# kylemcdonald/distributed-video-filter

Measured on AMD Instinct MI355X. Metric: frames/sec (1080p RGB invert) at 1/2/4/8 GPUs; kernel HBM GB/s vs peak, higher is better.
Workload: dtype u8; 1 GPU; configs[1]: 1080p RGB invert, batch=32, kernel-only, HBM-resident; global_batch=32, frames_per_rank_step=32, ring_bytes_in_plus_out=2388787200, kernel=invert_stream_kernel<4,nt,nt>, grid 32 WG/CU (vf_kernels.hip)

## Files before the change

### distributed-video-filter_amd/csrc/vf_jpeg.h

```cpp
#pragma once
#include <hip/hip_runtime.h>
#include <stddef.h>
#include <stdint.h>

#include "vf_jpeg_types.h"

namespace vf {
namespace jpeg {


hipError_t scan_u32(const ScanSeg *segs, int nseg, uint32_t max_tiles, const uint32_t *in, uint32_t *out,
                    uint32_t *tsum, uint32_t *totals, bool inclusive, hipStream_t s);
hipError_t scan_i32(const ScanSeg *segs, int nseg, uint32_t max_tiles, const int32_t *in, int32_t *out,
                    int32_t *tsum, int32_t *totals, bool inclusive, hipStream_t s);

hipError_t dec_unstuff_count(const DecSeg *sg, int nseg, uint32_t max_tiles, const uint8_t *in,
                             uint32_t *tile_cnt, hipStream_t s);
hipError_t dec_unstuff_write(const DecSeg *sg, int nseg, uint32_t max_tiles, const uint8_t *in,
                             const uint32_t *tile_off, const uint32_t *us_len, uint8_t *us, hipStream_t s);
hipError_t dec_syncg(int G, const DecSeg *sg, const DecFrame *fr, int nseg, uint32_t max_sub, const uint8_t *us,
                     const uint32_t *us_len, uint64_t *exits, uint32_t *cnts, uint64_t *used, uint64_t *ck,
                     uint32_t *ckrem, uint32_t *changed, int pass, uint32_t warm, int tabs4, hipStream_t s);
hipError_t dec_sync(const DecSeg *sg, const DecFrame *fr, int nseg, uint32_t max_sub, const uint8_t *us, const uint32_t *us_len,
                    const uint64_t *exit_in, uint64_t *exit_out, const uint32_t *cnt_in, uint32_t *cnt_out,
                    uint64_t *used, uint64_t *ck, uint32_t *ckrem, uint32_t *changed, int pass, hipStream_t s);
struct SpecBufs {
  uint64_t *tE;
  uint64_t *tX;
  uint32_t *tXc;
  uint64_t *pX;
  uint32_t *pC;
  uint8_t *wF;
  uint8_t *rE;
  uint32_t *rK;
  uint64_t *qX;
  uint32_t *qC;
  uint8_t *rL;
  uint32_t *stats;
};
constexpr int kSpecLanesMax = 16;
inline uint32_t spec_lanes_host(int bpm) { return bpm <= 1 ? 1u : bpm <= 2 ? 2u : bpm <= 4 ? 4u : bpm <= 8 ? 8u : 16u; }
hipError_t dec_sync_spec(const DecSeg *sg, const DecFrame *fr, int nseg, uint32_t max_wg, const uint8_t *us, const uint32_t *us_len,
                         const SpecBufs &b, uint64_t *exit_out, uint32_t *cnt_out, uint32_t *unresolved,
                         int lsb, hipStream_t s);
hipError_t dec_write(const DecSeg *sg, const DecFrame *fr, int nseg, uint32_t max_sub, const uint8_t *us, const uint32_t *us_len,
                     const uint64_t *exits, const uint32_t *bstart, int16_t *coef, int32_t *dcseq,
                     uint8_t *nmask, hipStream_t s);
hipError_t dec_write4(const DecSeg *sg, const DecFrame *fr, int nseg, uint32_t max_sub, const uint8_t *us,
                      const uint32_t *us_len, const uint64_t *exits, const uint32_t *cnt, const uint64_t *ck,
                      const uint32_t *ckrem, const uint32_t *bstart, int16_t *coef, int32_t *dcseq, uint8_t *nmask,
                      hipStream_t s);
hipError_t dec_idct(const DecFrame *fr, int n, uint32_t max_blocks, const int16_t *coef, const int32_t *dcseq,
                    const uint8_t *nmask, uint8_t *planes, hipStream_t s);
struct LutTable {
  uint32_t w[192];
};
hipError_t dec_color(const DecFrame *fr, int n, int max_w, int max_h, const uint8_t *planes, uint8_t *pix,
                     int bgr, int invert, const EncFrame *efr, int cm, hipStream_t s, const LutTable *lut = nullptr);
hipError_t dec_idct_color422(const DecFrame *fr, int n, int max_w, int max_h, const int16_t *coef,
                             const int32_t *dcseq, const uint8_t *nmask, uint8_t *eplanes, const EncFrame *efr,
                             int invert, int one_row,
                             hipStream_t s,
                             const LutTable *lut = nullptr);

hipError_t enc_fdct(const EncFrame *fr, int n, uint32_t max_blocks, const EncTables *tab, const uint8_t *pix,
                    int16_t *dcq, uint32_t *acbits, uint32_t *acscr, int bgr, int fastdct, int ch, int cv, int planes,
                    hipStream_t s);
hipError_t enc_len(const EncFrame *fr, int n, uint32_t max_blocks, const EncTables *tab, const int16_t *dcq,
                   uint32_t *acbits, uint32_t *bits, uint32_t *pre, hipStream_t s);
hipError_t enc_pack(const EncFrame *fr, int n, uint32_t max_blocks, const uint32_t *pre, const uint32_t *acbits,
                    const uint32_t *acscr, const uint32_t *bitoff, const uint32_t *total_bits, uint8_t *stream,
                    hipStream_t s);
hipError_t enc_ff_count(const EncFrame *fr, int n, uint32_t max_tiles, const uint32_t *total_bits,
                        const uint8_t *stream, uint32_t *tile_cnt, hipStream_t s);
hipError_t enc_ff_write(const EncFrame *fr, int n, uint32_t max_tiles, const uint32_t *total_bits,
                        const uint8_t *stream, const uint32_t *tile_off, const uint32_t *nff,
                        const uint8_t *hdr, uint8_t *pack, uint64_t *out_size, hipStream_t s);

}
}
```

### distributed-video-filter_amd/csrc/vf_jpeg_codec.h

```cpp
#pragma once
#include <hip/hip_runtime.h>

#include <atomic>
#include <condition_variable>
#include <functional>
#include <memory>
#include <mutex>
#include <string>
#include <thread>
#include <vector>

#include "vf_chain_plan.h"
#include "vf_jpeg.h"
#include "vf_jpeg_plan.h"

namespace vf {
namespace jpeg {

constexpr int kOk = 0;
constexpr int kInvalid = -1;
constexpr int kHip = -2;
constexpr int kNoMem = -3;
constexpr int kJpeg = -5;
constexpr int kResync = -100;

constexpr int kFlagFastUpsample = 256;
constexpr int kFlagFastDct = 2048;

struct DevBuf {
  void *p = nullptr;
  size_t cap = 0;
  hipError_t ensure(size_t n);
  template <typename T>
  T *as() const {
    return static_cast<T *>(p);
  }
  ~DevBuf();
};

struct HostBuf {
  void *p = nullptr;
  size_t cap = 0;
  hipError_t ensure(size_t n);
  template <typename T>
  T *as() const {
    return static_cast<T *>(p);
  }
  ~HostBuf();
};

class TaskPool {
 public:
  explicit TaskPool(int nthreads);
  ~TaskPool();
  TaskPool(const TaskPool &) = delete;
  TaskPool &operator=(const TaskPool &) = delete;
  void run(int n, const std::function<void(int)> &fn);

 private:
  void loop();
  void drain();
  std::vector<std::thread> threads_;
  std::mutex mu_;
  std::condition_variable cv_, done_cv_;
  uint64_t gen_ = 0;
  bool stop_ = false;
  int active_ = 0;
  int n_ = 0;
  std::atomic<int> next_{0};
  const std::function<void(int)> *fn_ = nullptr;
};

struct ComputeGate {
  std::mutex mu;
  hipEvent_t last = nullptr;
};

struct ChainSpec {
  chain::Program prog;
  std::vector<uint64_t> masks;
  chain::Buffers bufs;
};

struct Filter {
  enum Kind { kNone, kInvert, kTable, kChain } kind = kInvert;
  LutTable lut = {};
  std::shared_ptr<const ChainSpec> chain;
  bool in_colour() const { return kind == kInvert || kind == kTable; }
  bool between() const { return kind == kChain; }
};

int header_info(const uint8_t *jpeg, size_t size, int *w, int *h, int *subsamp, int *colorspace, std::string *err);
size_t buffer_size(int w, int h, int subsamp);

class Codec {
 public:
  explicit Codec(int device, ComputeGate *gate = nullptr);
  ~Codec();
  Codec(const Codec &) = delete;
  Codec &operator=(const Codec &) = delete;

  int encode(const uint8_t *const *imgs, const int *ws, const int *hs, int n, int pixel_format, int quality,
             int subsamp, int flags, uint8_t *const *outs, const size_t *caps, size_t *sizes, std::string *err);
  int decode(const uint8_t *const *jpegs, const size_t *sizes, int n, int pixel_format, int flags,
             uint8_t *const *outs, const size_t *caps, std::string *err);
  int invert(const uint8_t *const *jpegs, const size_t *sizes, int n, int quality, int subsamp, int flags,
             uint8_t *const *outs, const size_t *caps, size_t *out_sizes, const Filter &filter, std::string *err);
  int submit_invert(const uint8_t *const *jpegs, const size_t *sizes, int n, int quality, int subsamp, int flags,
                    const Filter &filter, std::string *err);
  bool done_invert();
  int wait_invert(size_t *total, std::string *err);
  int fetch_invert(uint8_t *out, size_t cap, size_t *sizes, size_t *offs, std::string *err);
  int scatter_invert(uint8_t *const *outs, const size_t *caps, size_t *sizes, int *placed);
  uint64_t fetch_refills() const { return fetch_refills_; }
  void set_max_pixels(uint64_t v) { max_pixels_ = v ? v : kDefaultMaxPixels; }
  bool waited() const { return waited_; }
  void quiesce();
  int bench_invert(const uint8_t *const *jpegs, const size_t *sizes, int n, int quality, int subsamp, int flags,
                   int iters, const Filter &filter, float *ms, float *stage_ms, std::string *err);

 private:
  int init(std::string *err);
  int prepare_decode(const uint8_t *const *jpegs, const size_t *sizes, int n, int flags, const JpegSwitches &sw,
                     std::string *err);
  int run_decode(int bgr, std::string *err);
  int run_decode_post(int bgr, std::string *err);
  hipError_t span_pass(int p);
  int finish_sync(std::string *err);
  int check_decode(std::string *err);
  template <class Tail>
  int settle_decode(int bgr, Tail &&tail, std::string *err);
  int prepare_encode(const int *ws, const int *hs, const uint64_t *img_offs, int n, int quality, int subsamp,
                     bool fastdct, std::string *err);
  int run_encode(int bgr, bool fastdct, const uint8_t *pix, std::string *err);
  int run_filter_encode(bool fastdct, std::string *err);
  int queue_fetch(uint64_t guess, std::string *err);
  int finish_fetch(std::string *err);
  int copy_out(uint8_t *const *outs, const size_t *caps, size_t *sizes, std::string *err);

  int device_;
  ComputeGate *gate_;
  uint64_t max_pixels_ = kDefaultMaxPixels;
  hipStream_t s_ = nullptr;
  hipEvent_t ev_[10] = {};
  bool stage_events_ = false;
  hipError_t stage_event(int i) { return stage_events_ ? hipEventRecord(ev_[i], s_) : hipSuccess; }
  hipEvent_t done_ = nullptr;

  HostBuf h_dfr_;
  DecFrame *dfr_ = nullptr;
  int ntabs_ = 0;
  std::vector<DecSeg> dsg_;
  std::vector<const uint8_t *> seg_src_;
  int dn_ = 0, dnseg_ = 0, ndcseg_ = 0;
  uint32_t dmax_tiles_ = 0, dmax_sub_ = 0, dmax_blocks_ = 0, dc_max_tiles_ = 0;
  int dmax_w_ = 0, dmax_h_ = 0;
  uint64_t dblocks_ = 0, dpix_bytes_ = 0;
  uint32_t dmax_wg_ = 0;
  uint64_t spec_calls_ = 0, spec_fallbacks_ = 0;
  DevBuf d_tE_, d_tX_, d_tXc_, d_pX_, d_pC_, d_wF_, d_rE_, d_rK_, d_qX_, d_qC_, d_rL_,
      d_unres_;
  int sync_passes_ = 0;
  DevBuf d_in_, d_dfr_, d_dsg_, d_segs_, d_tile_, d_tsum_, d_totals_, d_us_, d_exit_[2], d_cnt_[2], d_used_, d_ck_, d_ckrem_, d_bstart_,
      d_changed_, d_coef_, d_nmask_, d_dcseq_, d_dcpred_, d_planes_, d_pix_;

  std::vector<EncFrame> efr_;
  int en_ = 0;
  int esub_ = 1;
  uint32_t emax_blocks_ = 0, emax_tiles_ = 0;
  uint64_t eblocks_ = 0, ebits_bytes_ = 0;
  DevBuf d_eplanes_;
  Filter filter_;
  DevBuf d_pix2_;
  std::vector<std::unique_ptr<DevBuf>> d_chain_;
  int dcm_ = -1;
  DevBuf d_efr_, d_etab_, d_hdr_, d_esegs_, d_etsum_, d_etotals_, d_dcq_, d_acbits_, d_acscr_, d_bits_, d_pre_, d_bitoff_, d_stream_, d_ffcnt_,
      d_outsize_, d_pack_;

  HostBuf h_unres_;
  void *unres_dev_ = nullptr, *dtot_dev_ = nullptr;
  HostBuf h_stage_, h_out_, h_flag_;
  HostBuf h_ddesc_, h_edesc_, h_meta_, h_dtot_;
  uint64_t guess_ = 0, out_total_ = 0, fetch_refills_ = 0;
  bool waited_ = false;
  std::vector<uint64_t> out_sizes_, out_offs_;
  bool spec_check_ = false;
  bool pass_check_ = false;
  DecodePlan plan_;
  int sync_slot_ = 0;
  double out_ratio_ = 0;
  uint64_t in_bytes_ = 0;
  TaskPool pool_{4};
  double prep_ms_[3] = {0, 0, 0};
  std::vector<uint64_t> ekey_;
  bool ekey_valid_ = false;
  uint64_t enc_prep_reused_ = 0;
};

}
}
```

### distributed-video-filter_amd/csrc/vf_jpeg_host.hip

```cpp
#include <hip/hip_runtime.h>

#include <algorithm>
#include <chrono>
#include <cstdio>
#include <cstdlib>
#include <cstring>
#include <new>
#include <string>
#include <vector>

#include "vf_host_mem.h"
#include "vf_internal.h"
#include "vf_jpeg.h"
#include "vf_jpeg_codec.h"
#include "vf_jpeg_parse.h"
#include "vf_jpeg_plan.h"

namespace vf {
namespace jpeg {

namespace {


size_t write_header(int w, int h, int quality, int subsamp, uint8_t *o) {
  size_t n = 0;
  auto b = [&](int v) { o[n++] = (uint8_t)v; };
  auto u16 = [&](int v) {
    b(v >> 8);
    b(v & 0xFF);
  };
  const int nc = subsamp == 3 ? 1 : 3;
  uint16_t q[2][64];
  quality_table(quality, false, q[0]);
  quality_table(quality, true, q[1]);
  b(0xFF);
  b(0xD8);
  const uint8_t app0[18] = {0xFF, 0xE0, 0, 16, 'J', 'F', 'I', 'F', 0, 1, 1, 0, 0, 1, 0, 1, 0, 0};
  for (uint8_t v : app0) b(v);
  for (int t = 0; t < (nc == 3 ? 2 : 1); ++t) {
    b(0xFF);
    b(0xDB);
    u16(67);
    b(t);
    for (int i = 0; i < 64; ++i) b(q[t][kNatH[i]]);
  }
  b(0xFF);
  b(0xC0);
  u16(8 + 3 * nc);
  b(8);
  u16(h);
  u16(w);
  b(nc);
  for (int c = 0; c < nc; ++c) {
    b(c + 1);
    b(c == 0 ? (kSampH[subsamp] << 4) | kSampV[subsamp] : 0x11);
    b(c == 0 ? 0 : 1);
  }
  auto dht = [&](int idx, const uint8_t *bits, const uint8_t *vals) {
    int cnt = 0;
    for (int l = 1; l <= 16; ++l) cnt += bits[l];
    b(0xFF);
    b(0xC4);
    u16(19 + cnt);
    b(idx);
    for (int l = 1; l <= 16; ++l) b(bits[l]);
    for (int i = 0; i < cnt; ++i) b(vals[i]);
  };
  dht(0x00, kDcLBits, kDcVals);
  dht(0x10, kAcLBits, kAcLVals);
  if (nc == 3) {
    dht(0x01, kDcCBits, kDcVals);
    dht(0x11, kAcCBits, kAcCVals);
  }
  b(0xFF);
  b(0xDA);
  u16(6 + 2 * nc);
  b(nc);
  for (int c = 0; c < nc; ++c) {
    b(c + 1);
    b(c == 0 ? 0x00 : 0x11);
  }
  b(0);
  b(63);
  b(0);
  return n;
}

void build_enc_tables(int quality, bool fastdct, EncTables *t) {
  std::memset(t, 0, sizeof *t);
  for (int tb = 0; tb < 2; ++tb) {
    uint16_t q[64];
    quality_table(quality, tb == 1, q);
    for (int i = 0; i < 64; ++i) {
      const uint32_t divisor = fastdct ? (uint32_t)(((int32_t)q[i] * kAanScales[i] + (1 << 10)) >> 11)
                                       : (uint32_t)q[i] << 3;
      if (divisor == 1) {
        t->recip[tb][i] = 1;
        t->corr[tb][i] = 0;
        t->shift[tb][i] = -16;
        continue;
      }
      const int b = 31 - __builtin_clz(divisor);
      int r = 16 + b;
      uint32_t fq = (1u << r) / divisor, fr = (1u << r) % divisor, c = divisor / 2;
      if (fr == 0) {
        fq >>= 1;
        --r;
      } else if (fr <= divisor / 2u) {
        ++c;
      } else {
        ++fq;
      }
      t->recip[tb][i] = (uint16_t)fq;
      t->corr[tb][i] = (uint16_t)c;
      t->shift[tb][i] = (int16_t)(r - 16);
    }
  }
  for (int tb = 0; tb < 2; ++tb)
    for (int i = 0; i < 64; ++i) {
      uint32_t y = (uint32_t)(t->shift[tb][i] + 16);
      for (uint32_t j = 0; j < 4; ++j) y |= qo_pos(j, kZigOf[i]) << (8 + 6 * j);
      t->fdct_lds[2 * (64 * tb + i)] = (uint32_t)t->recip[tb][i] | ((uint32_t)t->corr[tb][i] << 16);
      t->fdct_lds[2 * (64 * tb + i) + 1] = y;
    }
  code_table(kDcLBits, kDcVals, t->dc[0], 16);
  code_table(kDcCBits, kDcVals, t->dc[1], 16);
  code_table(kAcLBits, kAcLVals, t->ac[0], 256);
  code_table(kAcCBits, kAcCVals, t->ac[1], 256);
  std::memcpy(t->fdct_lds + 256, t->ac, sizeof t->ac);
}

constexpr size_t kMaxBlockBytes = (27 + 63 * 26 + 7) / 8 + 1;

}



hipError_t DevBuf::ensure(size_t n) {
  if (n <= cap) return hipSuccess;
  if (p) (void)hipFree(p);
  p = nullptr;
  cap = 0;
  n = align_up(std::max<size_t>(n, 256), 1 << 20);
  hipError_t e = hipMalloc(&p, n);
  if (e == hipSuccess) cap = n;
  return e;
}

DevBuf::~DevBuf() {
  if (p) (void)hipFree(p);
}

hipError_t HostBuf::ensure(size_t n) {
  if (n <= cap) return hipSuccess;
  (void)numa_pinned_free(p);
  p = nullptr;
  cap = 0;
  n = align_up(std::max<size_t>(n, 256), 1 << 20);
  int dev = 0;
  (void)hipGetDevice(&dev);
  hipError_t e = numa_pinned_alloc(&p, n, device_numa_node(dev));
  if (e == hipSuccess) cap = n;
  return e;
}

HostBuf::~HostBuf() { (void)numa_pinned_free(p); }


TaskPool::TaskPool(int nthreads) {
  for (int i = 1; i < nthreads; ++i) threads_.emplace_back([this] { loop(); });
}

TaskPool::~TaskPool() {
  {
    std::lock_guard<std::mutex> lk(mu_);
    stop_ = true;
    ++gen_;
  }
  cv_.notify_all();
  for (auto &t : threads_) t.join();
}

void TaskPool::drain() {
  for (int i = next_.fetch_add(1); i < n_; i = next_.fetch_add(1)) (*fn_)(i);
}

void TaskPool::run(int n, const std::function<void(int)> &fn) {
  if (n <= 1 || threads_.empty()) {
    for (int i = 0; i < n; ++i) fn(i);
    return;
  }
  {
    std::lock_guard<std::mutex> lk(mu_);
    fn_ = &fn;
    n_ = n;
    next_.store(0);
    active_ = (int)threads_.size();
    ++gen_;
  }
  cv_.notify_all();
  drain();
  std::unique_lock<std::mutex> lk(mu_);
  done_cv_.wait(lk, [this] { return active_ == 0; });
  fn_ = nullptr;
}

void TaskPool::loop() {
  uint64_t seen = 0;
  for (;;) {
    {
      std::unique_lock<std::mutex> lk(mu_);
      cv_.wait(lk, [&] { return gen_ != seen; });
      seen = gen_;
      if (stop_) return;
    }
    drain();
    {
      std::lock_guard<std::mutex> lk(mu_);
      if (--active_ == 0) done_cv_.notify_one();
    }
  }
}

Codec::Codec(int device, ComputeGate *gate) : device_(device), gate_(gate) {}

Codec::~Codec() {
  (void)hipSetDevice(device_);
  if (s_) {
    (void)hipStreamSynchronize(s_);
    (void)hipStreamDestroy(s_);
  }
  for (hipEvent_t e : ev_)
    if (e) (void)hipEventDestroy(e);
  if (done_) (void)hipEventDestroy(done_);
}

#define CK(call)                                                                          \
  do {                                                                                    \
    hipError_t e_ = (call);                                                               \
    if (e_ != hipSuccess) {                                                               \
      *err = std::string(#call) + ": " + hipGetErrorString(e_);                           \
      return e_ == hipErrorOutOfMemory || e_ == hipErrorMemoryAllocation ? kNoMem : kHip; \
    }                                                                                     \
  } while (0)

int Codec::init(std::string *err) {
  if (s_) return kOk;
  CK(hipSetDevice(device_));
  CK(hipStreamCreateWithFlags(&s_, hipStreamNonBlocking));
  for (hipEvent_t &e : ev_) CK(hipEventCreate(&e));
  CK(hipEventCreateWithFlags(&done_, hipEventDisableTiming));
  return kOk;
}

int Codec::prepare_decode(const uint8_t *const *jpegs, const size_t *sizes, int n, int flags, const JpegSwitches &sw,
                          std::string *err) {
  if (n <= 0) {
    *err = "empty batch";
    return kInvalid;
  }
  const size_t toff = align_up(sizeof(DecFrame) * (size_t)n, 256);
  CK(h_dfr_.ensure(toff + sizeof(DecTabs) * (size_t)n));
  dfr_ = h_dfr_.as<DecFrame>();
  seg_src_.clear();
  std::vector<Parsed> parsed((size_t)n);
  uint64_t in_off = 0, us_off = 0, blk = 0, dcoff = 0, plane = 0, pix = 0;
  uint32_t tiles = 0, subs = 0, wgs = 0;
  uint64_t trs = 0;
  dmax_tiles_ = dmax_sub_ = dmax_blocks_ = dmax_wg_ = 0;
  BatchTraits traits;
  dmax_w_ = dmax_h_ = 0;
  std::vector<std::string> ferr((size_t)n);
  using clk = std::chrono::steady_clock;
  const auto tp0 = clk::now();
  std::vector<uint32_t> qmax((size_t)n);
  std::vector<uint64_t> khash((size_t)n);
  std::vector<std::vector<uint8_t>> keys((size_t)n);
  pool_.run(n, [&](int f) {
    Parsed &P = parsed[(size_t)f];
    std::string &e = ferr[(size_t)f];
    DecFrame &F = *new (&dfr_[(size_t)f]) DecFrame();
    parse_frame(jpegs[f], sizes[f], max_pixels_, &P, &F.g, nullptr, nullptr, nullptr, nullptr, nullptr, &e);
    if (!e.empty()) return;
    uint32_t q_ac = 0;
    for (int c = 0; c < P.ncomp; ++c) {
      std::memcpy(F.q[c], P.qt[P.tq[c]], sizeof F.q[c]);
      for (int i = 1; i < 64; ++i) q_ac = std::max(q_ac, (uint32_t)F.q[c][i]);
    }
    qmax[(size_t)f] = q_ac;
    khash[(size_t)f] = table_key(P, &keys[(size_t)f]);
  });
  const auto tp1 = clk::now();
  for (int f = 0; f < n; ++f)
    if (!ferr[(size_t)f].empty()) {
      *err = "frame " + std::to_string(f) + ": " + ferr[(size_t)f];
      return kJpeg;
    }
  std::vector<int> uniq;
  std::vector<int> acmax;
  std::vector<uint8_t> m24ok((size_t)n);
  for (int f = 0; f < n; ++f) {
    int u = 0;
    for (; u < (int)uniq.size(); ++u)
      if (khash[(size_t)uniq[(size_t)u]] == khash[(size_t)f] && keys[(size_t)uniq[(size_t)u]] == keys[(size_t)f]) break;
    if (u == (int)uniq.size()) {
      const Parsed &P = parsed[(size_t)f];
      DecTabs &T = *new (h_dfr_.as<uint8_t>() + toff + sizeof(DecTabs) * uniq.size()) DecTabs();
      for (int c = 0; c < P.ncomp; ++c)
        if (!build_tables(P.dcbits[P.td[c]], P.dcvals[P.td[c]], true, &T.dc[c], &T.sdc[c]) ||
            !build_tables(P.acbits[P.ta[c]], P.acvals[P.ta[c]], false, &T.ac[c], &T.sac[c], T.spair[c])) {
          *err = "frame " + std::to_string(f) + ": bad Huffman table";
          return kJpeg;
        }
      int a = 0;
      for (int c = 0; c < P.ncomp; ++c)
        for (int i = 0; i < 256; ++i) a = std::max(a, (int)(T.ac[c].vals[i] & 15));
      uniq.push_back(f);
      acmax.push_back(a);
    }
    dfr_[(size_t)f].tabs_off = toff + sizeof(DecTabs) * (size_t)u;
    m24ok[(size_t)f] = idct_col24_ok(acmax[(size_t)u], qmax[(size_t)f]) ? 1 : 0;
  }
  ntabs_ = (int)uniq.size();
  dsg_.clear();
  dcm_ = -2;
  const bool idct24 = flag_on(sw.idct24);
  for (int f = 0; f < n; ++f) {
    const Parsed &P = parsed[(size_t)f];
    DecFrame &F = dfr_[(size_t)f];
    F.flags = (flags & kFlagFastUpsample) ? 0u : 1u;
    {
      const Geom &g = F.g;
      uint32_t cm = 0;
      if (g.ncomp == 3 && g.he[0] == 1 && g.ve[0] == 1 && g.he[1] == g.he[2] && g.ve[1] == g.ve[2])
        cm = g.he[1] == 1 && g.ve[1] == 1 ? 1u : g.he[1] == 2 && g.ve[1] == 1 ? 2u : g.he[1] == 2 && g.ve[1] == 2 ? 3u : 0u;
      F.flags |= cm << 1;
      if (idct24 && m24ok[(size_t)f]) F.flags |= kDecIdct24;
      dcm_ = dcm_ == -2 || dcm_ == (int)cm ? (int)cm : -1;
      traits.d422 = traits.d422 && g.ncomp == 3 && g.hs[0] == 2 && g.vs[0] == 1 && g.hs[1] == 1 && g.vs[1] == 1 &&
              g.hs[2] == 1 && g.vs[2] == 1 && g.bpm == 4;
    }
    {
      uint32_t s4 = 0, rep = 0;
      int key[2] = {-1, -1}, nsl = 0;
      bool ok = true;
      for (int c = 0; c < P.ncomp && ok; ++c) {
        const int k = P.td[c] * 16 + P.ta[c];
        int sl = k == key[0] ? 0 : k == key[1] ? 1 : -1;
        if (sl < 0 && nsl == 2) ok = false;
        if (sl < 0 && ok) {
          key[nsl] = k;
          rep |= (uint32_t)c << (8 + 2 * nsl);
          sl = nsl++;
        }
        if (ok) s4 |= (uint32_t)sl << (2 * c);
      }
      if (ok && nsl == 1) rep |= (rep & 0x300u) << 2;
      F.tabs4 = ok ? (s4 | rep | 0x80000000u) : 0u;
      traits.tabs4 = traits.tabs4 && ok;
      traits.pow2bpm = traits.pow2bpm && F.g.bpm >= 1 && F.g.bpm <= 16 && (F.g.bpm & (F.g.bpm - 1)) == 0;
    }
    F.blk0 = blk;
    for (int c = 0; c < P.ncomp; ++c) {
      F.dcbase[c] = dcoff;
      dcoff += (uint64_t)F.g.nmcu * F.g.mh[c] * F.g.mv[c];
      F.plane_off[c] = plane;
      plane += align_up((size_t)F.g.pw[c] * F.g.ph[c], 256);
    }
    F.out_off = pix;
    pix += align_up((size_t)P.w * P.h * 3, 256);
    blk += (uint64_t)F.g.nblocks;
    const uint32_t nmcu = (uint32_t)F.g.nmcu, per = P.restart ? (uint32_t)P.restart : nmcu;
    size_t start = P.scan_off;
    for (size_t i = 0; i <= P.rst.size(); ++i) {
      const size_t end = i < P.rst.size() ? P.rst[i].first : P.scan_end;
      const size_t len = end - start;
      const uint32_t m0 = (uint32_t)i * per, mc = std::min(per, nmcu - m0);
      DecSeg S{};
      S.frame = (uint32_t)f;
      S.nblocks = mc * (uint32_t)F.g.bpm;
      S.blk0 = F.blk0 + (uint64_t)m0 * F.g.bpm;
      for (int c = 0; c < P.ncomp; ++c) S.dcbase[c] = F.dcbase[c] + (uint64_t)m0 * F.g.mh[c] * F.g.mv[c];
      S.in_off = in_off;
      S.in_len = (uint32_t)len;
      S.ntiles = (uint32_t)((len + kTile - 1) / kTile);
      S.tile0 = tiles;
      S.sub0 = subs;
      S.nsub_max = (uint32_t)((len * 8 + kSubBits - 1) / kSubBits);
      {
        const uint32_t ns = 256 / spec_lanes_host(F.g.bpm);
        S.nwg = S.nsub_max <= ns ? 1u : 1u + (S.nsub_max - ns + ns - 2) / (ns - 1);
        S.wg0 = wgs;
        S.tr0 = trs;
        wgs += S.nwg;
        trs += (uint64_t)S.nwg * 256;
        dmax_wg_ = std::max(dmax_wg_, S.nwg);
        if (S.nwg > 4096 || (uint64_t)S.nwg * (uint64_t)F.g.bpm > 16384) traits.spec_ok = false;
      }
      S.us_off = us_off;
      in_off += align_up(len, 16);
      us_off += align_up(len + 64, 16);
      tiles += S.ntiles;
      subs += S.nsub_max;
      dmax_tiles_ = std::max(dmax_tiles_, S.ntiles);
      dmax_sub_ = std::max(dmax_sub_, S.nsub_max);
      seg_src_.push_back(jpegs[f] + start);
      dsg_.push_back(S);
      if (i < P.rst.size()) start = P.rst[i].second + 2;
    }
    dmax_blocks_ = std::max(dmax_blocks_, (uint32_t)F.g.nblocks);
    dmax_w_ = std::max(dmax_w_, P.w);
    dmax_h_ = std::max(dmax_h_, P.h);
  }
  dn_ = n;
  dnseg_ = (int)dsg_.size();
  if (dnseg_ > 65535) {
    *err = "more than 65535 restart intervals in one batch (split the batch)";
    return kInvalid;
  }
  if (dcoff >= (1ull << 31)) {
    *err = "more than 2^31 blocks in one batch (split the batch)";
    return kInvalid;
  }
  dblocks_ = blk;
  dpix_bytes_ = pix;
  {
    uint64_t bits = 0;
    for (const DecSeg &S : dsg_) bits += (uint64_t)S.in_len * 8;
    traits.bits_per_block = blk ? bits / blk : 0;
  }
  std::vector<ScanSeg> segs;
  uint32_t t0 = 0;
  auto add = [&](uint64_t base, uint32_t len) {
    segs.push_back(ScanSeg{base, len, t0});
    t0 += (len + kScanTile - 1) / kScanTile;
  };
  for (auto &S : dsg_) add(S.tile0, S.ntiles);
  for (auto &S : dsg_) add(S.sub0, S.nsub_max);
  ndcseg_ = 0;
  dc_max_tiles_ = 0;
  for (auto &S : dsg_) {
    const Geom &g = dfr_[S.frame].g;
    for (int c = 0; c < g.ncomp; ++c) {
      const uint32_t len = S.nblocks / (uint32_t)g.bpm * (uint32_t)(g.mh[c] * g.mv[c]);
      add(S.dcbase[c], len);
      dc_max_tiles_ = std::max(dc_max_tiles_, (len + kScanTile - 1) / kScanTile);
      ++ndcseg_;
    }
  }
  const auto tp2 = clk::now();
  CK(h_stage_.ensure(in_off));
  pool_.run(dnseg_, [&](int i) {
    const DecSeg &S = dsg_[(size_t)i];
    std::memcpy(h_stage_.as<uint8_t>() + S.in_off, seg_src_[(size_t)i], S.in_len);
  });
  CK(hipSetDevice(device_));
  CK(d_in_.ensure(in_off));
  CK(d_dfr_.ensure(toff + sizeof(DecTabs) * (size_t)ntabs_));
  CK(d_dsg_.ensure(sizeof(DecSeg) * (size_t)dnseg_));
  CK(d_segs_.ensure(sizeof(ScanSeg) * segs.size()));
  CK(d_tile_.ensure(sizeof(uint32_t) * tiles));
  CK(d_tsum_.ensure(sizeof(int32_t) * (t0 + 1)));
  CK(d_totals_.ensure(sizeof(int32_t) * segs.size()));
  CK(h_dtot_.ensure(sizeof(uint32_t) * (size_t)dnseg_ + 64));
  CK(h_unres_.ensure(sizeof(uint32_t) * (size_t)dnseg_ + 64));
  CK(hipHostGetDevicePointer(&dtot_dev_, h_dtot_.p, 0));
  CK(hipHostGetDevicePointer(&unres_dev_, h_unres_.p, 0));
  CK(d_us_.ensure(us_off));
  CK(d_exit_[0].ensure(sizeof(uint64_t) * subs));
  CK(d_exit_[1].ensure(sizeof(uint64_t) * subs));
  CK(d_cnt_[0].ensure(sizeof(uint32_t) * subs));
  CK(d_cnt_[1].ensure(sizeof(uint32_t) * subs));
  CK(d_used_.ensure(sizeof(uint64_t) * subs));
  CK(d_ck_.ensure(sizeof(uint64_t) * subs * kCk));
  CK(d_ckrem_.ensure(sizeof(uint32_t) * subs * kCk));
  CK(d_bstart_.ensure(sizeof(uint32_t) * subs));
  {
    const size_t sl = (size_t)trs, wl = (size_t)wgs * kSpecLanesMax;
    CK(d_tE_.ensure(sizeof(uint64_t) * sl));
    CK(d_tX_.ensure(sizeof(uint64_t) * sl));
    CK(d_tXc_.ensure(sizeof(uint32_t) * sl));
    CK(d_pX_.ensure(sizeof(uint64_t) * sl));
    CK(d_pC_.ensure(sizeof(uint32_t) * sl));
    CK(d_wF_.ensure(wl));
    CK(d_rE_.ensure(wgs));
    CK(d_rK_.ensure(sizeof(uint32_t) * wgs));
    CK(d_qX_.ensure(sizeof(uint64_t) * sl));
    CK(d_qC_.ensure(sizeof(uint32_t) * sl));
    CK(d_rL_.ensure(wgs));
    CK(d_unres_.ensure(sizeof(uint32_t) * 16));
  }
  CK(d_changed_.ensure(sizeof(uint32_t) * kMaxPasses));
  CK(d_coef_.ensure(blk * 128));
  CK(d_nmask_.ensure(blk + 16));
  CK(d_dcseq_.ensure(sizeof(int32_t) * (dcoff + 1)));
  CK(d_dcpred_.ensure(sizeof(int32_t) * (dcoff + 1)));
  CK(d_planes_.ensure(plane));
  CK(d_pix_.ensure(pix));
  const size_t dsz = toff + sizeof(DecTabs) * (size_t)ntabs_, gsz = sizeof(DecSeg) * (size_t)dnseg_,
               ssz = sizeof(ScanSeg) * segs.size();
  CK(h_ddesc_.ensure(gsz + ssz));
  std::memcpy(h_ddesc_.as<uint8_t>(), dsg_.data(), gsz);
  std::memcpy(h_ddesc_.as<uint8_t>() + gsz, segs.data(), ssz);
  CK(hipMemcpyAsync(d_in_.p, h_stage_.p, in_off, hipMemcpyHostToDevice, s_));
  CK(hipMemcpyAsync(d_dfr_.p, h_dfr_.p, dsz, hipMemcpyHostToDevice, s_));
  CK(hipMemcpyAsync(d_dsg_.p, h_ddesc_.p, gsz, hipMemcpyHostToDevice, s_));
  CK(hipMemcpyAsync(d_segs_.p, h_ddesc_.as<uint8_t>() + gsz, ssz, hipMemcpyHostToDevice, s_));
  {
    auto ms = [](clk::time_point a, clk::time_point b) { return std::chrono::duration<double, std::milli>(b - a).count(); };
    prep_ms_[0] = ms(tp0, tp1);
    prep_ms_[1] = ms(tp1, tp2);
    prep_ms_[2] = ms(tp2, clk::now());
  }
  traits.max_sub = dmax_sub_;
  plan_ = resolve(sw, traits, filter_.in_colour());
  plan_.enc_fast = (flags & kFlagFastDct) != 0;
  return kOk;
}

int Codec::run_decode(int bgr, std::string *err) {
  const DecFrame *fr = d_dfr_.as<DecFrame>();
  const DecSeg *sg = d_dsg_.as<DecSeg>();
  const ScanSeg *segs = d_segs_.as<ScanSeg>();
  const int ns = dnseg_;
  CK(stage_event(0));
  CK(dec_unstuff_count(sg, ns, dmax_tiles_, d_in_.as<uint8_t>(), d_tile_.as<uint32_t>(), s_));
  uint32_t *us_len = d_totals_.as<uint32_t>();
  CK(scan_u32(segs, ns, (dmax_tiles_ + kScanTile - 1) / kScanTile, d_tile_.as<uint32_t>(), d_tile_.as<uint32_t>(),
              d_tsum_.as<uint32_t>(), us_len, false, s_));
  CK(dec_unstuff_write(sg, ns, dmax_tiles_, d_in_.as<uint8_t>(), d_tile_.as<uint32_t>(), us_len,
                       d_us_.as<uint8_t>(), s_));
  CK(stage_event(1));
  const DecodePlan &pl = plan_;
  int pass = 0;
  sync_slot_ = 0;
  if (pl.spec) {
    SpecBufs sb{d_tE_.as<uint64_t>(),  d_tX_.as<uint64_t>(), d_tXc_.as<uint32_t>(),
                d_pX_.as<uint64_t>(),  d_pC_.as<uint32_t>(), d_wF_.as<uint8_t>(),  d_rE_.as<uint8_t>(),
                d_rK_.as<uint32_t>(),  d_qX_.as<uint64_t>(), d_qC_.as<uint32_t>(), d_rL_.as<uint8_t>(),
                d_unres_.as<uint32_t>()};
    if (pl.stats) CK(hipMemsetAsync(d_unres_.p, 0, sizeof(uint32_t) * 16, s_));
    CK(dec_sync_spec(sg, fr, ns, dmax_wg_, d_us_.as<uint8_t>(), us_len, sb, d_exit_[0].as<uint64_t>(),
                     d_cnt_[0].as<uint32_t>(), static_cast<uint32_t *>(unres_dev_), pl.lsb ? 1 : 0, s_));
    spec_check_ = true;
    ++spec_calls_;
    if (pl.stats) {
      uint32_t st[16];
      CK(hipStreamSynchronize(s_));
      CK(hipMemcpy(st, d_unres_.p, sizeof st, hipMemcpyDeviceToHost));
      st[0] = 0;
      for (int i = 0; i < ns; ++i) st[0] += h_unres_.as<uint32_t>()[i];
      std::fprintf(stderr, "[vf_jpeg] k_spec phases (VF_SPEC_PHASES, 1024 wall ticks summed): part A %u, part B %u, "
                   "walkers end %u; walkers %u explicit rows %u rows written %u (workgroups %u)\n", st[8], st[9], st[10],
                   st[1], st[2], st[3], dmax_wg_ * (uint32_t)ns);
      std::fprintf(stderr, "[vf_jpeg] spec: unresolved %u; walk columns ended explicit %u, their traces joined in one "
                   "subsequence %u, serial traces %u (segments %d)\n", st[0], st[11], st[12], st[13], ns);
    }
  } else if (pl.g > 0) {
    CK(hipMemsetAsync(d_changed_.p, 0, sizeof(uint32_t) * kMaxPasses, s_));
    for (int p = 0; p < pl.queued; ++p) CK(span_pass(p));
    CK(h_flag_.ensure(64));
    CK(hipMemcpyAsync(h_flag_.p, d_changed_.as<uint32_t>() + pl.queued - 1, sizeof(uint32_t),
                      hipMemcpyDeviceToHost, s_));
    pass_check_ = true;
    pass = pl.queued;
  } else {
    CK(hipMemsetAsync(d_changed_.p, 0, sizeof(uint32_t) * kMaxPasses, s_));
    for (uint32_t flag = 1; flag;) {
      const int a = pass & 1;
      CK(dec_sync(sg, fr, ns, dmax_sub_, d_us_.as<uint8_t>(), us_len, d_exit_[a ^ 1].as<uint64_t>(),
                  d_exit_[a].as<uint64_t>(), d_cnt_[a ^ 1].as<uint32_t>(), d_cnt_[a].as<uint32_t>(),
                  d_used_.as<uint64_t>(), d_ck_.as<uint64_t>(), d_ckrem_.as<uint32_t>(),
                  d_changed_.as<uint32_t>() + (pass % kMaxPasses), pass > 0 ? 1 : 0, s_));
      sync_slot_ = a;
      ++pass;
      if (pass < 2) continue;
      CK(hipMemcpyAsync(&flag, d_changed_.as<uint32_t>() + ((pass - 1) % kMaxPasses), sizeof flag,
                        hipMemcpyDeviceToHost, s_));
      CK(hipStreamSynchronize(s_));
      if (!flag) break;
      CK(hipMemsetAsync(d_changed_.as<uint32_t>() + (pass % kMaxPasses), 0, sizeof(uint32_t), s_));
      if (pass > (int)dmax_sub_ + 2) {
        *err = "Huffman synchronisation did not converge (corrupt stream?)";
        return kJpeg;
      }
    }
  }
  sync_passes_ = pass;
  if (pl.stats) {
    uint32_t st[4];
    CK(hipMemcpy(st, d_changed_.as<uint32_t>() + kMaxPasses - 4, sizeof st, hipMemcpyDeviceToHost));
    std::fprintf(stderr,
                 "[vf_jpeg] sync: spec calls %llu fallbacks %llu; passes %d; rounds pass0 max %u sum %u, pass1 max %u "
                 "sum %u (WGs %u)\n",
                 (unsigned long long)spec_calls_, (unsigned long long)spec_fallbacks_, pass, st[3], st[1], st[2], st[0],
                 (dmax_sub_ + 255) / 256 * (uint32_t)ns);
  }
  CK(stage_event(2));
  return run_decode_post(bgr, err);
}

hipError_t Codec::span_pass(int p) {
  return dec_syncg(plan_.g, d_dsg_.as<DecSeg>(), d_dfr_.as<DecFrame>(), dnseg_, dmax_sub_, d_us_.as<uint8_t>(),
                   d_totals_.as<uint32_t>(), d_exit_[0].as<uint64_t>(), d_cnt_[0].as<uint32_t>(), d_used_.as<uint64_t>(),
                   d_ck_.as<uint64_t>(), d_ckrem_.as<uint32_t>(), d_changed_.as<uint32_t>(), p, plan_.warm, plan_.tabs,
                   s_);
}

int Codec::finish_sync(std::string *err) {
  for (int p = plan_.queued;; ++p) {
    if (p >= kMaxPasses) {
      *err = "Huffman synchronisation did not converge (corrupt stream?)";
      return kJpeg;
    }
    CK(span_pass(p));
    uint32_t flag = 0;
    CK(hipMemcpyAsync(&flag, d_changed_.as<uint32_t>() + p, sizeof flag, hipMemcpyDeviceToHost, s_));
    CK(hipStreamSynchronize(s_));
    if (!flag) break;
  }
  return kOk;
}

int Codec::run_decode_post(int bgr, std::string *err) {
  const DecFrame *fr = d_dfr_.as<DecFrame>();
  const DecSeg *sg = d_dsg_.as<DecSeg>();
  const ScanSeg *segs = d_segs_.as<ScanSeg>();
  const int n = dn_, ns = dnseg_;
  const uint32_t *us_len = d_totals_.as<uint32_t>();
  const DecodePlan &pl = plan_;
  const int last = sync_slot_;
  const bool invert = filter_.in_colour();
  const LutTable *const lut = filter_.kind == Filter::kTable ? &filter_.lut : nullptr;
  uint32_t *blocks_total = static_cast<uint32_t *>(dtot_dev_);
  CK(scan_u32(segs + ns, ns, (dmax_sub_ + kScanTile - 1) / kScanTile, d_cnt_[last].as<uint32_t>(),
              d_bstart_.as<uint32_t>(), d_tsum_.as<uint32_t>(), blocks_total, false, s_));
  uint8_t *const nmask = pl.chunks ? d_nmask_.as<uint8_t>() : nullptr;
  if (!pl.chunks) CK(hipMemsetAsync(d_coef_.p, 0, dblocks_ * 128, s_));
  if (!pl.spec && pl.write4)
    CK(dec_write4(sg, fr, ns, dmax_sub_, d_us_.as<uint8_t>(), us_len, d_exit_[last].as<uint64_t>(),
                  d_cnt_[last].as<uint32_t>(), d_ck_.as<uint64_t>(), d_ckrem_.as<uint32_t>(),
                  d_bstart_.as<uint32_t>(), d_coef_.as<int16_t>(), d_dcseq_.as<int32_t>(), nmask, s_));
  else
    CK(dec_write(sg, fr, ns, dmax_sub_, d_us_.as<uint8_t>(), us_len, d_exit_[last].as<uint64_t>(),
                 d_bstart_.as<uint32_t>(), d_coef_.as<int16_t>(), d_dcseq_.as<int32_t>(), nmask, s_));
  CK(stage_event(3));
  CK(scan_i32(segs + 2 * ns, ndcseg_, dc_max_tiles_, d_dcseq_.as<int32_t>(), d_dcpred_.as<int32_t>(),
              d_tsum_.as<int32_t>(), nullptr, true, s_));
  if (pl.fuse_idct) {
    CK(stage_event(4));
    CK(dec_idct_color422(fr, n, dmax_w_, dmax_h_, d_coef_.as<int16_t>(), d_dcpred_.as<int32_t>(), nmask,
                         d_eplanes_.as<uint8_t>(), d_efr_.as<EncFrame>(), invert ? 1 : 0, kSampV[esub_] == 1 ? 1 : 0,
                         s_, lut));
    CK(stage_event(5));
    return kOk;
  }
  CK(dec_idct(fr, n, dmax_blocks_, d_coef_.as<int16_t>(), d_dcpred_.as<int32_t>(), nmask, d_planes_.as<uint8_t>(), s_));
  CK(stage_event(4));
  CK(dec_color(fr, n, dmax_w_, dmax_h_, d_planes_.as<uint8_t>(), pl.fuse ? d_eplanes_.as<uint8_t>() : d_pix_.as<uint8_t>(),
               bgr, invert ? 1 : 0, pl.fuse ? d_efr_.as<EncFrame>() : nullptr, dcm_, s_, lut));
  CK(stage_event(5));
  return kOk;
}

int Codec::check_decode(std::string *err) {
  const uint32_t *tot = h_dtot_.as<uint32_t>();
  if (pass_check_) {
    pass_check_ = false;
    if (*h_flag_.as<uint32_t>()) return kResync;
  }
  if (spec_check_) {
    spec_check_ = false;
    bool unresolved = false;
    for (int i = 0; i < dnseg_; ++i) unresolved = unresolved || h_unres_.as<uint32_t>()[i] != 0;
    if (unresolved) {
      ++spec_fallbacks_;
      *err = "speculative Huffman synchronisation left a frame unresolved";
      return kJpeg;
    }
  }
  for (int i = 0; i < dnseg_; ++i) {
    const DecSeg &S = dsg_[(size_t)i];
    if (tot[(size_t)i] < S.nblocks) {
      const bool whole = S.nblocks == (uint32_t)dfr_[S.frame].g.nblocks;
      *err = "frame " + std::to_string(S.frame) + (whole ? std::string() : " (restart interval at block " +
             std::to_string(S.blk0 - dfr_[S.frame].blk0) + ")") + ": entropy-coded data ends after " +
             std::to_string(tot[(size_t)i]) + " of " + std::to_string(S.nblocks) + " blocks (truncated or corrupt JPEG)";
      return kJpeg;
    }
  }
  return kOk;
}

int Codec::prepare_encode(const int *ws, const int *hs, const uint64_t *img_offs, int n, int quality, int subsamp,
                          bool fastdct, std::string *err) {
  if (subsamp < 0 || subsamp > 4) {
    *err = "unsupported subsampling (TJSAMP_444, 422, 420, GRAY, 440)";
    return kInvalid;
  }
  {
    std::vector<uint64_t> key;
    key.reserve(3 * (size_t)n + 4);
    key.push_back((uint64_t)n);
    key.push_back((uint64_t)quality);
    key.push_back((uint64_t)subsamp);
    key.push_back(fastdct ? 1u : 0u);
    for (int f = 0; f < n; ++f) {
      key.push_back((uint64_t)(uint32_t)ws[f] << 32 | (uint32_t)hs[f]);
      key.push_back(img_offs[f]);
    }
    if (ekey_valid_ && key == ekey_) {
      ++enc_prep_reused_;
      return kOk;
    }
    ekey_valid_ = false;
    ekey_.swap(key);
  }
  efr_.assign((size_t)n, EncFrame());
  std::vector<uint8_t> hdr;
  uint64_t blk = 0, bits = 0, out = 0, epl = 0;
  uint32_t tiles = 0;
  emax_blocks_ = emax_tiles_ = 0;
  const int nc = subsamp == 3 ? 1 : 3;
  const int hsamp[3] = {kSampH[subsamp], 1, 1}, vsamp[3] = {kSampV[subsamp], 1, 1};
  for (int f = 0; f < n; ++f) {
    EncFrame &F = efr_[(size_t)f];
    if (!make_geom(ws[f], hs[f], nc, hsamp, vsamp, &F.g)) {
      *err = "frame " + std::to_string(f) + ": bad image size";
      return kInvalid;
    }
    F.img_off = img_offs[f];
    for (int k = 0; k < 3; ++k) {
      F.eplane_off[k] = epl;
      if (k < nc) epl += align_up((size_t)F.g.wb[k] * 8 * (size_t)F.g.rrows[k], 256);
    }
    F.blk0 = blk;
    F.bits_off = bits;
    const uint64_t bits_cap = align_up((size_t)F.g.nblocks * kMaxBlockBytes + 16, 256);
    F.out_off = out;
    F.hdr_off = (uint32_t)hdr.size();
    uint8_t h[1024];
    F.hdr_len = (uint32_t)write_header(ws[f], hs[f], quality, subsamp, h);
    hdr.insert(hdr.end(), h, h + F.hdr_len);
    F.tile0 = tiles;
    F.ntiles_max = (uint32_t)((bits_cap + kTile - 1) / kTile);
    blk += (uint64_t)F.g.nblocks;
    bits += bits_cap;
    out += align_up(F.hdr_len + 2 * bits_cap + 2, 256);
    tiles += F.ntiles_max;
    emax_blocks_ = std::max(emax_blocks_, (uint32_t)F.g.nblocks);
    emax_tiles_ = std::max(emax_tiles_, F.ntiles_max);
  }
  en_ = n;
  esub_ = subsamp;
  eblocks_ = blk;
  ebits_bytes_ = bits;
  std::vector<ScanSeg> segs;
  uint32_t t0 = 0;
  auto add = [&](uint64_t base, uint32_t len) {
    segs.push_back(ScanSeg{base, len, t0});
    t0 += (len + kScanTile - 1) / kScanTile;
  };
  for (auto &F : efr_) add(F.blk0, (uint32_t)F.g.nblocks);
  for (auto &F : efr_) add(F.tile0, F.ntiles_max);
  EncTables tab;
  build_enc_tables(quality, fastdct, &tab);
  CK(hipSetDevice(device_));
  CK(d_efr_.ensure(sizeof(EncFrame) * (size_t)n));
  CK(d_etab_.ensure(sizeof(EncTables)));
  CK(d_hdr_.ensure(hdr.size()));
  CK(d_esegs_.ensure(sizeof(ScanSeg) * segs.size()));
  CK(d_etsum_.ensure(sizeof(uint32_t) * (t0 + 1)));
  CK(d_etotals_.ensure(sizeof(uint32_t) * segs.size()));
  CK(d_dcq_.ensure(sizeof(int16_t) * blk));
  CK(d_acbits_.ensure(sizeof(uint32_t) * blk));
  CK(d_acscr_.ensure(sizeof(uint32_t) * kAcScratchWords * ((blk + 63) & ~(size_t)63)));
  CK(d_bits_.ensure(sizeof(uint32_t) * blk));
  CK(d_pre_.ensure(sizeof(uint32_t) * blk));
  CK(d_bitoff_.ensure(sizeof(uint32_t) * blk));
  CK(d_stream_.ensure(bits));
  CK(d_ffcnt_.ensure(sizeof(uint32_t) * tiles));
  CK(d_pack_.ensure(out));
  CK(d_outsize_.ensure(sizeof(uint64_t) * (size_t)n));
  CK(d_eplanes_.ensure(epl));
  const size_t fsz = sizeof(EncFrame) * (size_t)n, ssz = sizeof(ScanSeg) * segs.size();
  const size_t o_tab = align_up(fsz, 256), o_hdr = o_tab + align_up(sizeof tab, 256),
               o_seg = o_hdr + align_up(hdr.size(), 256);
  CK(h_edesc_.ensure(o_seg + ssz));
  uint8_t *hb = h_edesc_.as<uint8_t>();
  std::memcpy(hb, efr_.data(), fsz);
  std::memcpy(hb + o_tab, &tab, sizeof tab);
  std::memcpy(hb + o_hdr, hdr.data(), hdr.size());
  std::memcpy(hb + o_seg, segs.data(), ssz);
  CK(hipMemcpyAsync(d_efr_.p, hb, fsz, hipMemcpyHostToDevice, s_));
  CK(hipMemcpyAsync(d_etab_.p, hb + o_tab, sizeof tab, hipMemcpyHostToDevice, s_));
  CK(hipMemcpyAsync(d_hdr_.p, hb + o_hdr, hdr.size(), hipMemcpyHostToDevice, s_));
  CK(hipMemcpyAsync(d_esegs_.p, hb + o_seg, ssz, hipMemcpyHostToDevice, s_));
  ekey_valid_ = true;
  return kOk;
}

int Codec::run_filter_encode(bool fastdct, std::string *err) {
  if (!filter_.between()) return run_encode(1, fastdct, d_pix_.as<uint8_t>(), err);
  const ChainSpec &c = *filter_.chain;
  while ((int)d_chain_.size() + 2 < c.bufs.count) d_chain_.emplace_back(new DevBuf());
  std::vector<uint8_t *> base((size_t)c.bufs.count), at((size_t)c.bufs.count);
  for (int k = 0; k < c.bufs.count; ++k) {
    DevBuf &b = k == 0 ? d_pix_ : k == 1 ? d_pix2_ : *d_chain_[(size_t)k - 2];
    if (k != 0) CK(b.ensure(dpix_bytes_));
    base[(size_t)k] = b.as<uint8_t>();
  }
  const LaunchCfg cfg;
  std::vector<chain::Launch> launches;
  int launches_h = -1;
  for (int f = 0; f < dn_; ++f) {
    const DecFrame &F = dfr_[(size_t)f];
    const int h = F.g.h;
    if (h != launches_h) launches = chain::band_launches(c.prog, c.bufs, h, 0, h, 0, false);
    launches_h = h;
    for (size_t k = 0; k < base.size(); ++k) at[k] = base[k] + F.out_off;
    CK(run_launches(c.prog, c.masks.data(), launches, at.data(), nullptr, F.g.w, 3, h, 0, cfg, s_));
  }
  return run_encode(1, fastdct, base[(size_t)c.bufs.result], err);
}

int Codec::run_encode(int bgr, bool fastdct, const uint8_t *pix, std::string *err) {
  const EncFrame *fr = d_efr_.as<EncFrame>();
  const EncTables *tab = d_etab_.as<EncTables>();
  const ScanSeg *segs = d_esegs_.as<ScanSeg>();
  const int n = en_;
  const bool fuse = plan_.fuse;
  CK(stage_event(6));
  CK(enc_fdct(fr, n, emax_blocks_, tab, fuse ? d_eplanes_.as<uint8_t>() : pix, d_dcq_.as<int16_t>(),
              d_acbits_.as<uint32_t>(), d_acscr_.as<uint32_t>(), bgr, fastdct ? 1 : 0, kSampH[esub_], kSampV[esub_],
              fuse ? 1 : 0, s_));
  CK(enc_len(fr, n, emax_blocks_, tab, d_dcq_.as<int16_t>(), d_acbits_.as<uint32_t>(), d_bits_.as<uint32_t>(),
             d_pre_.as<uint32_t>(), s_));
  uint32_t *total_bits = d_etotals_.as<uint32_t>();
  CK(scan_u32(segs, n, (emax_blocks_ + kScanTile - 1) / kScanTile, d_bits_.as<uint32_t>(), d_bitoff_.as<uint32_t>(),
              d_etsum_.as<uint32_t>(), total_bits, false, s_));
  CK(enc_pack(fr, n, emax_blocks_, d_pre_.as<uint32_t>(), d_acbits_.as<uint32_t>(), d_acscr_.as<uint32_t>(),
              d_bitoff_.as<uint32_t>(), total_bits, d_stream_.as<uint8_t>(), s_));
  CK(stage_event(7));
  CK(enc_ff_count(fr, n, emax_tiles_, total_bits, d_stream_.as<uint8_t>(), d_ffcnt_.as<uint32_t>(), s_));
  uint32_t *nff = d_etotals_.as<uint32_t>() + n;
  CK(scan_u32(segs + n, n, (emax_tiles_ + kScanTile - 1) / kScanTile, d_ffcnt_.as<uint32_t>(),
              d_ffcnt_.as<uint32_t>(), d_etsum_.as<uint32_t>(), nff, false, s_));
  CK(enc_ff_write(fr, n, emax_tiles_, total_bits, d_stream_.as<uint8_t>(), d_ffcnt_.as<uint32_t>(), nff,
                  d_hdr_.as<uint8_t>(), d_pack_.as<uint8_t>(), d_outsize_.as<uint64_t>(), s_));
  CK(stage_event(8));
  return kOk;
}

int Codec::queue_fetch(uint64_t guess, std::string *err) {
  const int n = en_;
  CK(h_meta_.ensure(sizeof(uint64_t) * (size_t)n * 2 + 64));
  uint64_t *sz = h_meta_.as<uint64_t>() + n;
  CK(hipMemcpyAsync(sz, d_outsize_.p, sizeof(uint64_t) * (size_t)n, hipMemcpyDeviceToHost, s_));
  guess = std::min<uint64_t>(guess, d_pack_.cap);
  CK(h_out_.ensure(guess));
  guess_ = guess;
  if (guess) CK(hipMemcpyAsync(h_out_.p, d_pack_.p, guess, hipMemcpyDeviceToHost, s_));
  CK(hipEventRecord(done_, s_));
  return kOk;
}

int Codec::finish_fetch(std::string *err) {
  const int n = en_;
  const uint64_t *sz = h_meta_.as<uint64_t>() + n;
  out_sizes_.resize((size_t)n);
  out_offs_.resize((size_t)n);
  uint64_t total = 0;
  for (int f = 0; f < n; ++f) {
    out_sizes_[(size_t)f] = sz[f];
    out_offs_[(size_t)f] = total;
    total += align_up(sz[f], 64);
  }
  out_total_ = total;
  if (total > guess_) {
    ++fetch_refills_;
    if (total > h_out_.cap) {
      HostBuf bigger;
      CK(bigger.ensure(total));
      std::memcpy(bigger.p, h_out_.p, guess_);
      std::swap(bigger.p, h_out_.p);
      std::swap(bigger.cap, h_out_.cap);
    }
    CK(hipMemcpyAsync(h_out_.as<uint8_t>() + guess_, d_pack_.as<uint8_t>() + guess_, total - guess_,
                      hipMemcpyDeviceToHost, s_));
    CK(hipStreamSynchronize(s_));
  }
  return kOk;
}

template <class Tail>
int Codec::settle_decode(int bgr, Tail &&tail, std::string *err) {
  int rc = check_decode(err);
  while (rc == kResync) {
    if ((rc = finish_sync(err)) || (rc = run_decode_post(bgr, err)) || (rc = tail())) return rc;
    rc = check_decode(err);
  }
  return rc;
}


int Codec::encode(const uint8_t *const *imgs, const int *ws, const int *hs, int n, int pixel_format, int quality,
                  int subsamp, int flags, uint8_t *const *outs, const size_t *caps, size_t *sizes, std::string *err) {
  int rc = init(err);
  if (rc) return rc;
  if (n <= 0) return kOk;
  if (pixel_format != 0 && pixel_format != 1) {
    *err = "pixel_format must be TJPF_RGB (0) or TJPF_BGR (1)";
    return kInvalid;
  }
  std::vector<uint64_t> offs((size_t)n);
  uint64_t pix = 0;
  for (int f = 0; f < n; ++f) {
    if (!imgs[f] || ws[f] <= 0 || hs[f] <= 0 || ws[f] > 65535 || hs[f] > 65535) {
      *err = "frame " + std::to_string(f) + ": bad image";
      return kInvalid;
    }
    offs[(size_t)f] = pix;
    pix += align_up((size_t)ws[f] * hs[f] * 3, 256);
  }
  const bool fast = (flags & kFlagFastDct) != 0;
  if ((rc = prepare_encode(ws, hs, offs.data(), n, quality, subsamp, fast, err))) return rc;
  plan_ = DecodePlan();
  filter_ = Filter{};
  CK(h_stage_.ensure(pix));
  CK(d_pix_.ensure(pix));
  pool_.run(n, [&](int f) {
    std::memcpy(h_stage_.as<uint8_t>() + offs[(size_t)f], imgs[f], (size_t)ws[f] * hs[f] * 3);
  });
  CK(hipMemcpyAsync(d_pix_.p, h_stage_.p, pix, hipMemcpyHostToDevice, s_));
  if ((rc = run_encode(pixel_format, fast, d_pix_.as<uint8_t>(), err))) return rc;
  uint64_t guess = 0;
  for (int f = 0; f < n; ++f) guess += align_up((size_t)ws[f] * hs[f] / 4 + 8192, 64);
  if ((rc = queue_fetch(guess, err))) return rc;
  CK(hipEventSynchronize(done_));
  if ((rc = finish_fetch(err))) return rc;
  return copy_out(outs, caps, sizes, err);
}

int Codec::copy_out(uint8_t *const *outs, const size_t *caps, size_t *sizes, std::string *err) {
  const int n = en_;
  for (int f = 0; f < n; ++f) {
    sizes[f] = (size_t)out_sizes_[(size_t)f];
    if (out_sizes_[(size_t)f] > caps[f] || !outs[f]) {
      *err = "frame " + std::to_string(f) + ": output buffer of " + std::to_string(caps[f]) +
             " bytes is too small for the " + std::to_string(out_sizes_[(size_t)f]) + "-byte JPEG";
      return kInvalid;
    }
  }
  pool_.run(n, [&](int f) {
    std::memcpy(outs[f], h_out_.as<uint8_t>() + out_offs_[(size_t)f], out_sizes_[(size_t)f]);
  });
  return kOk;
}

int Codec::decode(const uint8_t *const *jpegs, const size_t *jsizes, int n, int pixel_format, int flags,
                  uint8_t *const *outs, const size_t *caps, std::string *err) {
  int rc = init(err);
  if (rc) return rc;
  if (n <= 0) return kOk;
  if (pixel_format != 0 && pixel_format != 1) {
    *err = "pixel_format must be TJPF_RGB (0) or TJPF_BGR (1)";
    return kInvalid;
  }
  filter_.kind = Filter::kNone;
  if ((rc = prepare_decode(jpegs, jsizes, n, flags, JpegSwitches::read(), err))) return rc;
  for (int f = 0; f < n; ++f) {
    const size_t need = (size_t)dfr_[(size_t)f].g.w * dfr_[(size_t)f].g.h * 3;
    if (!outs[f] || caps[f] < need) {
      *err = "frame " + std::to_string(f) + ": output buffer smaller than " + std::to_string(need) + " bytes";
      return kInvalid;
    }
  }
  if ((rc = run_decode(pixel_format, err))) return rc;
  auto fetch_pixels = [&]() -> int {
    CK(h_out_.ensure(dpix_bytes_));
    CK(hipMemcpyAsync(h_out_.p, d_pix_.p, dpix_bytes_, hipMemcpyDeviceToHost, s_));
    CK(hipStreamSynchronize(s_));
    return kOk;
  };
  if ((rc = fetch_pixels()) || (rc = settle_decode(pixel_format, fetch_pixels, err))) return rc;
  pool_.run(n, [&](int f) {
    std::memcpy(outs[f], h_out_.as<uint8_t>() + dfr_[(size_t)f].out_off,
                (size_t)dfr_[(size_t)f].g.w * dfr_[(size_t)f].g.h * 3);
  });
  return kOk;
}

int Codec::submit_invert(const uint8_t *const *jpegs, const size_t *jsizes, int n, int quality, int subsamp,
                         int flags, const Filter &filter, std::string *err) {
  int rc = init(err);
  if (rc) return rc;
  waited_ = false;
  filter_ = filter;
  if (n <= 0) {
    *err = "empty batch";
    return kInvalid;
  }
  const JpegSwitches sw = JpegSwitches::read();
  using clk = std::chrono::steady_clock;
  const auto t0 = clk::now();
  if ((rc = prepare_decode(jpegs, jsizes, n, flags, sw, err))) return rc;
  const auto t1 = clk::now();
  std::vector<int> ws((size_t)n), hs((size_t)n);
  std::vector<uint64_t> offs((size_t)n);
  const double ratio = flag_on(sw.fetch_learn) ? out_ratio_ : 0.0;
  uint64_t guess = 0;
  in_bytes_ = 0;
  for (int f = 0; f < n; ++f) {
    ws[(size_t)f] = dfr_[(size_t)f].g.w;
    hs[(size_t)f] = dfr_[(size_t)f].g.h;
    offs[(size_t)f] = dfr_[(size_t)f].out_off;
    in_bytes_ += jsizes[f];
    guess += ratio > 0 ? align_up((uint64_t)((double)jsizes[f] * ratio * 1.06) + 1024, 64)
                       : align_up(jsizes[f] + jsizes[f] / 4 + 8192, 64);
  }
  if ((rc = prepare_encode(ws.data(), hs.data(), offs.data(), n, quality, subsamp, plan_.enc_fast, err))) return rc;
  const auto t2 = clk::now();
  {
    std::unique_lock<std::mutex> gl;
    if (gate_) {
      gl = std::unique_lock<std::mutex>(gate_->mu);
      if (gate_->last) CK(hipStreamWaitEvent(s_, gate_->last, 0));
    }
    if ((rc = run_decode(1, err))) return rc;
    if ((rc = run_filter_encode(plan_.enc_fast, err))) return rc;
    if (gate_) {
      CK(hipEventRecord(ev_[9], s_));
      gate_->last = ev_[9];
    }
  }
  if ((rc = queue_fetch(guess, err))) return rc;
  if (plan_.trace) {
    auto ms = [](clk::time_point a, clk::time_point b) { return std::chrono::duration<double, std::milli>(b - a).count(); };
    static const clk::time_point origin = t0;
    std::fprintf(stderr, "[vf_jpeg] submit codec %p n=%d at %.3f: prep_dec %.3f (parse %.3f loop %.3f stage %.3f) "
                 "prep_enc %.3f queue %.3f ms\n", (void *)this, n, ms(origin, t0), ms(t0, t1), prep_ms_[0], prep_ms_[1],
                 prep_ms_[2], ms(t1, t2), ms(t2, clk::now()));
  }
  return kOk;
}

void Codec::quiesce() {
  if (!s_) return;
  (void)hipSetDevice(device_);
  (void)hipStreamSynchronize(s_);
  (void)hipGetLastError();
}

bool Codec::done_invert() {
  const hipError_t q = hipEventQuery(done_);
  if (q == hipSuccess) return true;
  (void)hipGetLastError();
  return q != hipErrorNotReady;
}

int Codec::wait_invert(size_t *total, std::string *err) {
  using clk = std::chrono::steady_clock;
  const auto t0 = clk::now();
  CK(hipEventSynchronize(done_));
  int rc = settle_decode(1, [&]() -> int {
    int r = run_filter_encode(plan_.enc_fast, err);
    if (!r) r = queue_fetch(guess_, err);
    if (r) return r;
    CK(hipEventSynchronize(done_));
    return kOk;
  }, err);
  if (rc) return rc;
  if ((rc = finish_fetch(err))) return rc;
  if (in_bytes_) out_ratio_ = (double)out_total_ / (double)in_bytes_;
  waited_ = true;
  *total = (size_t)out_total_;
  if (plan_.trace)
    std::fprintf(stderr, "[vf_jpeg] wait codec %p: %.3f ms, %llu B fetched (%s)\n", (void *)this,
                 std::chrono::duration<double, std::milli>(clk::now() - t0).count(),
                 (unsigned long long)out_total_, out_total_ > guess_ ? "second copy" : "one copy");
  return kOk;
}

int Codec::scatter_invert(uint8_t *const *outs, const size_t *caps, size_t *sizes, int *placed) {
  const int n = en_;
  int count = 0;
  for (int f = 0; f < n; ++f) {
    sizes[f] = (size_t)out_sizes_[(size_t)f];
    count += outs[f] && out_sizes_[(size_t)f] <= caps[f];
  }
  pool_.run(n, [&](int f) {
    if (outs[f] && out_sizes_[(size_t)f] <= caps[f])
      std::memcpy(outs[f], h_out_.as<uint8_t>() + out_offs_[(size_t)f], out_sizes_[(size_t)f]);
  });
  *placed = count;
  return kOk;
}

int Codec::fetch_invert(uint8_t *out, size_t cap, size_t *sizes, size_t *offs, std::string *err) {
  const int n = en_;
  if (out && cap < out_total_) {
    *err = "output buffer of " + std::to_string(cap) + " bytes is smaller than the " +
           std::to_string(out_total_) + " packed bytes";
    return kInvalid;
  }
  for (int f = 0; f < n; ++f) {
    if (sizes) sizes[f] = (size_t)out_sizes_[(size_t)f];
    if (offs) offs[f] = (size_t)out_offs_[(size_t)f];
  }
  if (out && out_total_) {
    constexpr int kParts = 8;
    const uint64_t per = align_up((out_total_ + kParts - 1) / kParts, 4096);
    pool_.run(kParts, [&](int i) {
      const uint64_t b = std::min<uint64_t>(out_total_, per * (uint64_t)i);
      const uint64_t e = std::min<uint64_t>(out_total_, b + per);
      if (e > b) std::memcpy(out + b, h_out_.as<uint8_t>() + b, e - b);
    });
  }
  return kOk;
}

int Codec::invert(const uint8_t *const *jpegs, const size_t *jsizes, int n, int quality, int subsamp, int flags,
                  uint8_t *const *outs, const size_t *caps, size_t *sizes, const Filter &filter, std::string *err) {
  if (n <= 0) return init(err);
  int rc = submit_invert(jpegs, jsizes, n, quality, subsamp, flags, filter, err);
  size_t total = 0;
  if (!rc) rc = wait_invert(&total, err);
  if (!rc) rc = copy_out(outs, caps, sizes, err);
  return rc;
}

int Codec::bench_invert(const uint8_t *const *jpegs, const size_t *jsizes, int n, int quality, int subsamp,
                        int flags, int iters, const Filter &filter, float *ms, float *stage_ms, std::string *err) {
  int rc = init(err);
  if (rc) return rc;
  if (n <= 0 || iters <= 0) {
    *err = "bench_invert: empty batch or iters <= 0";
    return kInvalid;
  }
  filter_ = filter;
  if ((rc = prepare_decode(jpegs, jsizes, n, flags, JpegSwitches::read(), err))) return rc;
  std::vector<int> ws((size_t)n), hs((size_t)n);
  std::vector<uint64_t> offs((size_t)n);
  for (int f = 0; f < n; ++f) {
    ws[(size_t)f] = dfr_[(size_t)f].g.w;
    hs[(size_t)f] = dfr_[(size_t)f].g.h;
    offs[(size_t)f] = dfr_[(size_t)f].out_off;
  }
  const bool fast = plan_.enc_fast;
  if ((rc = prepare_encode(ws.data(), hs.data(), offs.data(), n, quality, subsamp, fast, err))) return rc;
  float acc[8] = {0};
  double total_ms = 0;
  int passes = 0;
  for (int pass = 0; pass < (stage_ms ? 2 : 1); ++pass) {
    stage_events_ = pass == 1;
    for (int it = 0; it < iters; ++it) {
      CK(hipStreamSynchronize(s_));
      const auto t0 = std::chrono::steady_clock::now();
      if ((rc = run_decode(1, err)) || (rc = run_filter_encode(fast, err))) {
        stage_events_ = false;
        return rc;
      }
      CK(hipStreamSynchronize(s_));
      if (pass == 0) {
        total_ms += std::chrono::duration<double, std::milli>(std::chrono::steady_clock::now() - t0).count();
        passes += sync_passes_;
        continue;
      }
      const int pairs[7][2] = {{0, 1}, {1, 2}, {2, 3}, {3, 4}, {4, 5}, {6, 7}, {7, 8}};
      for (int i = 0; i < 7; ++i) {
        float t = 0.f;
        if (hipEventElapsedTime(&t, ev_[pairs[i][0]], ev_[pairs[i][1]]) == hipSuccess) acc[i] += t;
      }
    }
  }
  stage_events_ = false;
  CK(hipStreamSynchronize(s_));
  rc = settle_decode(1, [&]() -> int {
    const int r = run_filter_encode(fast, err);
    if (r) return r;
    CK(hipStreamSynchronize(s_));
    return kOk;
  }, err);
  if (rc) return rc;
  *ms = (float)(total_ms / iters);
  if (stage_ms) {
    for (int i = 0; i < 7; ++i) stage_ms[i] = acc[i] / iters;
    stage_ms[7] = (float)passes / iters;
  }
  return kOk;
}

int header_info(const uint8_t *jpeg, size_t size, int *w, int *h, int *subsamp, int *colorspace, std::string *err) {
  Parsed P;
  if (!jpeg || parse(jpeg, size, &P, err, false) != 0) {
    if (!jpeg) *err = "NULL JPEG buffer";
    return kJpeg;
  }
  *w = P.w;
  *h = P.h;
  *subsamp = subsamp_of(P);
  *colorspace = P.ncomp == 1 ? 2 : 1;
  return kOk;
}

size_t buffer_size(int w, int h, int subsamp) {
  if (w <= 0 || h <= 0 || subsamp < 0 || subsamp > 4) return 0;
  const int nc = subsamp == 3 ? 1 : 3;
  const int hsamp[3] = {kSampH[subsamp], 1, 1}, vsamp[3] = {kSampV[subsamp], 1, 1};
  Geom g;
  if (!make_geom(w, h, nc, hsamp, vsamp, &g)) return 0;
  return 1024 + 2 * (size_t)g.nblocks * kMaxBlockBytes + 2;
}

}
}
```

### distributed-video-filter_amd/csrc/vf_jpeg_kernels.hip

```cpp
#include <hip/hip_runtime.h>
#include <stddef.h>
#include <stdint.h>

#include <type_traits>

#include "vf_jpeg.h"

namespace vf {
namespace jpeg {

namespace {

__device__ __forceinline__ uint32_t bswap32(uint32_t x) { return __builtin_bswap32(x); }

template <typename T>
__device__ __forceinline__ T wave_incl_scan(T x) {
  const int lane = threadIdx.x & 63;
#pragma unroll
  for (int o = 1; o < 64; o <<= 1) {
    const T y = __shfl_up(x, o, 64);
    if (lane >= o) x += y;
  }
  return x;
}
// ... 1543 lines not shown
  z4 = tmp1 + tmp3;
  z5 = imul<M24>(z3 + z4, FIX_1_175875602);
  tmp0 = imul<M24>(tmp0, FIX_0_298631336);
  tmp1 = imul<M24>(tmp1, FIX_2_053119869);
  tmp2 = imul<M24>(tmp2, FIX_3_072711026);
  tmp3 = imul<M24>(tmp3, FIX_1_501321110);
  z1 = imul<M24>(z1, -FIX_0_899976223);
  z2 = imul<M24>(z2, -FIX_2_562915447);
  z3 = imul<M24>(z3, -FIX_1_961570560);
  z4 = imul<M24>(z4, -FIX_0_390180644);
  z3 += z5;
  z4 += z5;
  tmp0 += z1 + z3;
  tmp1 += z2 + z4;
  tmp2 += z2 + z3;
  tmp3 += z1 + z4;
  emit(0, tmp10 + tmp3);
  emit(7, tmp10 - tmp3);
  emit(1, tmp11 + tmp2);
  emit(6, tmp11 - tmp2);
  emit(2, tmp12 + tmp1);
  emit(5, tmp12 - tmp1);
  emit(3, tmp13 + tmp0);
  emit(4, tmp13 - tmp0);
}
template <bool M24>
__device__ __forceinline__ void idct_line(const int32_t in[8], int32_t out[8], int shift) {
  const int32_t r = (int32_t)1 << (shift - 1);
  idct_core<M24>(in, [&](int i, int32_t v) { out[i] = (v + r) >> shift; });
}

__device__ __forceinline__ void idct_row_limited(const int32_t in[8], uint32_t out[8]) {
  idct_core<true>(in, [&](int i, int32_t v) {
    const int32_t m = (int32_t)__builtin_amdgcn_ubfe((uint32_t)v + ((1u << 17) + (512u << 18)), 18, 10) - 384;
    out[i] = (uint32_t)min(max(m, 0), 255);
  });
}

constexpr int kIdctNb = 2;
constexpr int kIdctBlocks = 32 * kIdctNb;

__constant__ uint8_t kIdctPos[64] = {
    1,  0,  9,  17, 8,  3,  2,  11, 16, 25, 32, 27, 19, 10, 5,  4,  12, 18, 26, 34, 42, 48,
    40, 33, 29, 21, 14, 7,  6,  13, 20, 24, 35, 46, 51, 56, 57, 49, 41, 38, 31, 23, 15, 22,
    28, 36, 43, 50, 58, 59, 52, 44, 37, 30, 39, 45, 54, 60, 61, 53, 47, 55, 62, 63};
__constant__ uint32_t kIdctCol[8] = {
    0x00201111u, 0x13023000u, 0x21612333u, 0x32135222u, 0x44360545u, 0x56447464u, 0x65554757u, 0x77776676u};

constexpr uint32_t kIdctGroup = 8 * kIdctNb;
__global__ __launch_bounds__(256) void k_idct(const DecFrame *__restrict__ fr, const int16_t *coef, const int32_t *dcseq,
                                              const uint8_t *nmask, uint8_t *planes) {
  const DecFrame &F = fr[blockIdx.y];
  const Geom &g = F.g;
  const uint32_t bpm = (uint32_t)g.bpm, nmcu = (uint32_t)g.nmcu;
  const uint32_t ngroups = (nmcu + kIdctGroup - 1) / kIdctGroup;
  if (blockIdx.x * 4 >= ngroups * bpm) return;
  __shared__ int32_t blkv[kIdctBlocks][72];
  __shared__ int32_t s_q[3][72];
  __shared__ uint8_t s_pos[64];
  __shared__ uint32_t s_col[8];
  const uint32_t t = threadIdx.x;
  const uint32_t slot = t >> 3, r = t & 7, lm = slot & 7;
  const uint32_t unit = blockIdx.x * 4 + __builtin_amdgcn_readfirstlane(t >> 6);
  const uint32_t grp = unit / bpm, c = unit - grp * bpm;
  const bool live = grp < ngroups;
  const uint32_t k = live ? (uint32_t)g.bcomp[c] : 0u;
  const uint32_t mh = (uint32_t)g.mh[k], mv = (uint32_t)g.mv[k], mcux = (uint32_t)g.mcux;
  const uint32_t mx0 = (grp * kIdctGroup) % mcux, my0 = (grp * kIdctGroup) / mcux;
  bool valid[kIdctNb];
  uint32_t bxs[kIdctNb], bys[kIdctNb];
  uint4 raw[kIdctNb];
  int32_t dc[kIdctNb];
  uint32_t nm[kIdctNb];
#pragma unroll
  for (int h = 0; h < kIdctNb; ++h) {
    const uint32_t mcu = grp * kIdctGroup + h * 8 + lm;
    valid[h] = live && mcu < nmcu;
    uint32_t mx = mx0 + h * 8 + lm, my = my0;
    while (mx >= mcux) mx -= mcux, ++my;
    bxs[h] = mx * mh + (uint32_t)g.bxo[c];
    bys[h] = my * mv + (uint32_t)g.byo[c];
    const uint64_t bi = valid[h] ? F.blk0 + (uint64_t)mcu * bpm + c : F.blk0;
    const uint64_t di = valid[h] ? F.dcbase[k] + (uint64_t)mcu * (mh * mv) + (c - (uint32_t)g.cfirst[k]) : F.dcbase[k];
    raw[h] = *reinterpret_cast<const uint4 *>(coef + bi * 64 + r * 8);
    dc[h] = dcseq[di];
    nm[h] = nmask ? (uint32_t)nmask[bi] : 0xFFu;
  }
  if (t < 192) s_q[t >> 6][t & 63] = F.q[t >> 6][t & 63];
  if (t < 64) s_pos[t] = kIdctPos[t];
  if (t < 8) s_col[t] = kIdctCol[t];
  __syncthreads();
  uint8_t *const plane = planes + F.plane_off[k];
  const uint32_t pw = (uint32_t)g.pw[k];
  const uint2 pos8 = *reinterpret_cast<const uint2 *>(&s_pos[r * 8]);
  const uint32_t colg = s_col[r];
#pragma unroll
  for (int h = 0; h < kIdctNb; ++h) {
    if (!valid[h]) continue;
    const bool st = (nm[h] >> r) & 1;
    const uint32_t qw[4] = {st ? raw[h].x : 0u, st ? raw[h].y : 0u, st ? raw[h].z : 0u, st ? raw[h].w : 0u};
#pragma unroll
    for (int j = 0; j < 8; ++j) {
      const int32_t v = (int32_t)(int16_t)(qw[j >> 1] >> (16 * (j & 1)));
      const uint32_t at = ((j < 4 ? pos8.x : pos8.y) >> (8 * (j & 3))) & 0xFF;
      blkv[h * 32 + slot][at] = (r == 0 && j == 0) ? (int32_t)(int16_t)dc[h] : v;
    }
  }
  __syncthreads();
  int32_t col[kIdctNb][8];
  const auto pass1 = [&](auto m24) {
#pragma unroll
    for (int h = 0; h < kIdctNb; ++h) {
      if (!valid[h]) continue;
      int32_t in[8];
#pragma unroll
      for (int i = 0; i < 8; ++i)
        in[i] = __mul24(blkv[h * 32 + slot][i * 8 + ((colg >> (4 * i)) & 7)], s_q[k][i * 8 + r]);
      idct_line<decltype(m24)::value>(in, col[h], 11);
    }
  };
  if (F.flags & kDecIdct24) pass1(BoolTag<true>{});
  else pass1(BoolTag<false>{});
  __syncthreads();
#pragma unroll
  for (int h = 0; h < kIdctNb; ++h) {
    if (!valid[h]) continue;
#pragma unroll
    for (int i = 0; i < 8; ++i) blkv[h * 32 + slot][i * 9 + r] = col[h][i];
  }
  __syncthreads();
#pragma unroll
  for (int h = 0; h < kIdctNb; ++h) {
    if (!valid[h]) continue;
    int32_t in[8];
    uint32_t out[8];
#pragma unroll
    for (int i = 0; i < 8; ++i) in[i] = blkv[h * 32 + slot][r * 9 + i];
    idct_row_limited(in, out);
    uint32_t lo = 0, hi = 0;
#pragma unroll
    for (int i = 0; i < 4; ++i) {
      lo |= out[i] << (8 * i);
      hi |= out[i + 4] << (8 * i);
    }
    uint8_t *p = plane + (uint64_t)(bys[h] * 8 + r) * pw + bxs[h] * 8;
    *reinterpret_cast<uint2 *>(p) = make_uint2(lo, hi);
  }
}


__device__ __forceinline__ int up_sample(const uint8_t *p, int pw, int dw, int dh, int he, int ve, bool fancy,
                                         int x, int y) {
  if (he == 1 && ve == 1) return p[(size_t)y * pw + x];
  const int iy = y / ve < dh ? y / ve : dh - 1;
  if (!fancy) return p[(size_t)iy * pw + x / he];
  const uint8_t *r0 = p + (size_t)iy * pw;
  if (he == 2 && ve == 1) {
    const int i = x >> 1;
    if (!(x & 1)) return i == 0 ? r0[0] : (3 * r0[i] + r0[i - 1] + 1) >> 2;
    return i == dw - 1 ? r0[i] : (3 * r0[i] + r0[i + 1] + 2) >> 2;
  }
  int ny = (y & 1) ? iy + 1 : iy - 1;
  ny = ny < 0 ? 0 : ny > dh - 1 ? dh - 1 : ny;
  const uint8_t *r1 = p + (size_t)ny * pw;
  if (he == 1) return (3 * r0[x] + r1[x] + ((y & 1) ? 2 : 1)) >> 2;
  const int i = x >> 1;
  const int t = 3 * r0[i] + r1[i];
  if (!(x & 1)) return i == 0 ? (4 * t + 8) >> 4 : (3 * t + 3 * r0[i - 1] + r1[i - 1] + 8) >> 4;
  return i == dw - 1 ? (4 * t + 7) >> 4 : (3 * t + 3 * r0[i + 1] + r1[i + 1] + 7) >> 4;
}

__device__ __forceinline__ uint32_t clamp255(int v) { return (uint32_t)(v < 0 ? 0 : v > 255 ? 255 : v); }

__device__ __forceinline__ void up2(const int cs[6], int i0, int dw, bool fancy, int ve, int out[8]) {
#pragma unroll
  for (int jj = 0; jj < 4; ++jj) {
    const int i = i0 + jj, c = cs[jj + 1];
    int a, b;
    if (!fancy) {
      a = b = c;
    } else if (ve == 1) {
      a = i == 0 ? c : (3 * c + cs[jj] + 1) >> 2;
      b = i == dw - 1 ? c : (3 * c + cs[jj + 2] + 2) >> 2;
    } else {
      a = i == 0 ? (4 * c + 8) >> 4 : (3 * c + cs[jj] + 8) >> 4;
      b = i == dw - 1 ? (4 * c + 7) >> 4 : (3 * c + cs[jj + 2] + 7) >> 4;
    }
    out[2 * jj] = a;
    out[2 * jj + 1] = b;
  }
}

template <bool LUT = false>
__device__ __forceinline__ void ycc8(const int v[3][8], int ncomp, int bgr, int invert, uint8_t o[24],
                                     const uint8_t *lut = nullptr) {
#pragma unroll
  for (int j = 0; j < 8; ++j) {
    uint32_t r, gg, b;
    if (ncomp == 1) {
      r = gg = b = (uint32_t)v[0][j];
    } else {
      const int xcr = v[2][j] - 128, xcb = v[1][j] - 128;
      r = clamp255(v[0][j] + ((__mul24(91881, xcr) + 32768) >> 16));
      gg = clamp255(v[0][j] + ((__mul24(-22554, xcb) + 32768 - __mul24(46802, xcr)) >> 16));
      b = clamp255(v[0][j] + ((__mul24(116130, xcb) + 32768) >> 16));
    }
    if constexpr (LUT) {
      r = lut[512 + r];
      gg = lut[256 + gg];
      b = lut[b];
    } else if (invert) {
      r ^= 0xFF;
      gg ^= 0xFF;
      b ^= 0xFF;
    }
    o[3 * j] = (uint8_t)(bgr ? b : r);
    o[3 * j + 1] = (uint8_t)gg;
    o[3 * j + 2] = (uint8_t)(bgr ? r : b);
  }
}

__device__ __forceinline__ void unpack8(uint2 q, int v[8]) {
#pragma unroll
  for (int j = 0; j < 8; ++j) v[j] = (int)(((j < 4 ? q.x : q.y) >> (8 * (j & 3))) & 0xFF);
}

template <bool LUT = false>
__device__ __forceinline__ void color8(const DecFrame &F, const Geom &g, const uint8_t *__restrict__ planes, int y,
                                       int x0, int bgr, int invert, uint8_t o[24], const uint8_t *lut = nullptr) {
  int v[3][8];
#pragma unroll
  for (int k = 0; k < 3; ++k) {
    if (k >= g.ncomp) break;
    const uint8_t *p = planes + F.plane_off[k];
    const int pw = g.pw[k];
    const int he = g.he[k], ve = g.ve[k], dw = g.dw[k], dh = g.dh[k];
    const bool fancy = (F.flags & 1) && ((he == 2 && dw > 2) || (he == 1 && ve == 2));
    if (he == 1 && ve == 1) {
      const uint2 q = *reinterpret_cast<const uint2 *>(p + (size_t)y * pw + x0);
#pragma unroll
      for (int j = 0; j < 8; ++j) v[k][j] = (int)(((j < 4 ? q.x : q.y) >> (8 * (j & 3))) & 0xFF);
    } else if (he == 2 && ve <= 2) {
      const int iy = min(y / ve, dh - 1);
      const uint8_t *r0 = p + (size_t)iy * pw;
      const int i0 = x0 >> 1;
      int cs[6];
      if (ve == 2 && fancy) {
        int ny = (y & 1) ? iy + 1 : iy - 1;
        ny = ny < 0 ? 0 : ny > dh - 1 ? dh - 1 : ny;
        const uint8_t *r1 = p + (size_t)ny * pw;
#pragma unroll
        for (int m = 0; m < 6; ++m) {
          const int ix = min(max(i0 - 1 + m, 0), dw - 1);
          cs[m] = 3 * r0[ix] + r1[ix];
        }
      } else {
#pragma unroll
        for (int m = 0; m < 6; ++m) cs[m] = r0[min(max(i0 - 1 + m, 0), dw - 1)];
      }
      up2(cs, i0, dw, fancy, ve, v[k]);
    } else {
#pragma unroll
      for (int j = 0; j < 8; ++j)
        v[k][j] = up_sample(p, pw, dw, dh, he, ve, fancy && he <= 2 && ve <= 2, min(x0 + j, g.w - 1), y);
    }
  }
  ycc8<LUT>(v, g.ncomp, bgr, invert, o, lut);
}

struct Ycc {
  int a0, a1, a2, bias;
};
__device__ __forceinline__ Ycc ycc_coefs(int k, bool bgr) {
  int r, g, b, bias = (128 << 16) + 32767;
  if (k == 0) {
    r = 19595, g = 38470, b = 7471, bias = 32768;
  } else if (k == 1) {
    r = -11059, g = -21709, b = 32768;
  } else {
    r = 32768, g = -27439, b = -5329;
  }
  return bgr ? Ycc{b, g, r, bias} : Ycc{r, g, b, bias};
}
__device__ __forceinline__ int ycc_apply(const Ycc &q, int c0, int c1, int c2) {
  return (__mul24(q.a0, c0) + __mul24(q.a1, c1) + __mul24(q.a2, c2) + q.bias) >> 16;
}

typedef short vf_i16x2 __attribute__((ext_vector_type(2)));
struct EncCoef {
  uint32_t sel, sh;
  vf_i16x2 c;
  int m, bias;
};
__device__ __forceinline__ EncCoef enc_coef(int k) {
  if (k == 0) return EncCoef{0x0C020C00u, 8u, vf_i16x2{19595, 7471}, 38470, 32768};
  if (k == 1) return EncCoef{0x0C010C00u, 16u, vf_i16x2{-11059, -21709}, 32768, (128 << 16) + 32767};
  return EncCoef{0x0C020C01u, 0u, vf_i16x2{-27439, -5329}, 32768, (128 << 16) + 32767};
}
__device__ __forceinline__ int enc_sample(uint32_t px, const EncCoef &q) {
  const vf_i16x2 pr = __builtin_bit_cast(vf_i16x2, __builtin_amdgcn_perm(px, px, q.sel));
  return __builtin_amdgcn_sdot2(pr, q.c, __mul24((int)((px >> q.sh) & 0xFF), q.m) + q.bias, false) >> 16;
}

template <bool ONE = false>
__device__ __forceinline__ void enc_store_rows(const EncFrame &E, uint8_t *__restrict__ eplanes, uint32_t (&p0)[8],
                                               uint32_t (&p1)[8], int y0, int x0, int w) {
  const Geom &ge = E.g;
  const bool edge = x0 + 8 >= w;
  uint32_t l0 = 0, l1 = 0;
  if (edge) {
    const int lp = w - 1 - x0;
#pragma unroll
    for (int p = 0; p < 8; ++p) {
      l0 = p == lp ? p0[p] : l0;
      l1 = p == lp ? p1[p] : l1;
    }
#pragma unroll
    for (int p = 0; p < 8; ++p) {
      p0[p] = p > lp ? l0 : p0[p];
      p1[p] = p > lp ? l1 : p1[p];
    }
  }
#pragma unroll 1
  for (int k = 0; k < ge.ncomp; ++k) {
    const int he = ge.he[k], ve = ge.ve[k], pitch = ge.wb[k] * 8, rr = ge.rrows[k];
    uint8_t *const pl = eplanes + E.eplane_off[k];
    const EncCoef q = enc_coef(k);
    int c0[8], c1[8];
#pragma unroll
    for (int p = 0; p < 8; ++p) c0[p] = enc_sample(p0[p], q), c1[p] = enc_sample(p1[p], q);
    const int e0 = edge ? enc_sample(l0, q) : 0, e1 = edge ? enc_sample(l1, q) : 0;
    if (ve == 1) {
#pragma unroll
      for (int rw = 0; rw < (ONE ? 1 : 2); ++rw) {
        const int y = y0 + rw;
        if (y >= rr) break;
        uint8_t *row = pl + (size_t)y * pitch;
        if (he == 1) {
          uint32_t lo = 0, hi = 0;
#pragma unroll
          for (int p = 0; p < 4; ++p) {
            lo |= (uint32_t)(rw ? c1[p] : c0[p]) << (8 * p);
            hi |= (uint32_t)(rw ? c1[p + 4] : c0[p + 4]) << (8 * p);
          }
#if VF_ABL & 8
          if (lo == 0x12345678u && hi == 0x9ABCDEF0u)
#endif
          *reinterpret_cast<uint2 *>(row + x0) = make_uint2(lo, hi);
        } else {
          uint32_t v = 0;
#pragma unroll
          for (int i = 0; i < 4; ++i)
            v |= (uint32_t)(((rw ? c1[2 * i] + c1[2 * i + 1] : c0[2 * i] + c0[2 * i + 1]) + (i & 1)) >> 1) << (8 * i);
#if VF_ABL & 8
          if (v == 0x12345678u)
#endif
          *reinterpret_cast<uint32_t *>(row + (x0 >> 1)) = v;
        }
        if (edge) {
          const int ev = rw ? e1 : e0;
          #pragma clang loop unroll(disable) vectorize(disable)
          for (int xs = (x0 + 8) / he; xs < pitch; ++xs) row[xs] = (uint8_t)ev;
        }
      }
    } else {
      const int y = y0 >> 1;
      if (y < rr) {
        uint8_t *row = pl + (size_t)y * pitch;
        if (he == 1) {
          uint32_t lo = 0, hi = 0;
#pragma unroll
          for (int p = 0; p < 4; ++p) {
            lo |= (uint32_t)((c0[p] + c1[p] + 1) >> 1) << (8 * p);
            hi |= (uint32_t)((c0[p + 4] + c1[p + 4] + 1) >> 1) << (8 * p);
          }
          *reinterpret_cast<uint2 *>(row + x0) = make_uint2(lo, hi);
          if (edge)
            #pragma clang loop unroll(disable) vectorize(disable)
            for (int xs = x0 + 8; xs < pitch; ++xs) row[xs] = (uint8_t)((e0 + e1 + 1) >> 1);
        } else {
          uint32_t v = 0;
#pragma unroll
          for (int i = 0; i < 4; ++i)
            v |= (uint32_t)((c0[2 * i] + c0[2 * i + 1] + c1[2 * i] + c1[2 * i + 1] + 1 + (i & 1)) >> 2) << (8 * i);
          *reinterpret_cast<uint32_t *>(row + (x0 >> 1)) = v;
          if (edge)
            #pragma clang loop unroll(disable) vectorize(disable)
            for (int xs = (x0 + 8) >> 1; xs < pitch; ++xs) row[xs] = (uint8_t)((2 * e0 + 2 * e1 + 1 + (xs & 1)) >> 2);
        }
      }
    }
  }
}

__device__ __forceinline__ void enc_sample_rows(const EncFrame &E, uint8_t *__restrict__ eplanes, const uint8_t o0[24],
                                                const uint8_t o1[24], int y0, int x0, int w, int bgr) {
  uint32_t p0[8], p1[8];
  const int i0 = bgr ? 2 : 0, i2 = bgr ? 0 : 2;
#pragma unroll
  for (int p = 0; p < 8; ++p) {
    p0[p] = (uint32_t)o0[3 * p + i0] | (uint32_t)o0[3 * p + 1] << 8 | (uint32_t)o0[3 * p + i2] << 16;
    p1[p] = (uint32_t)o1[3 * p + i0] | (uint32_t)o1[3 * p + 1] << 8 | (uint32_t)o1[3 * p + i2] << 16;
  }
  enc_store_rows(E, eplanes, p0, p1, y0, x0, w);
}

__device__ __forceinline__ void store24(uint8_t *dst, int left, const uint8_t o[24]) {
  if (left >= 8 && ((uintptr_t)dst & 7) == 0) {
    uint2 *d2 = reinterpret_cast<uint2 *>(dst);
#pragma unroll
    for (int q = 0; q < 3; ++q) {
      uint32_t lo = 0, hi = 0;
#pragma unroll
      for (int j = 0; j < 4; ++j) {
        lo |= (uint32_t)o[8 * q + j] << (8 * j);
        hi |= (uint32_t)o[8 * q + 4 + j] << (8 * j);
      }
      d2[q] = make_uint2(lo, hi);
    }
  } else {
    const int n = min(8, left) * 3;
    for (int j = 0; j < n; ++j) dst[j] = o[j];
  }
}


struct GlobalPlanes {
  const uint8_t *__restrict__ planes;
  const DecFrame &F;
  __device__ __forceinline__ const uint8_t *row(int k, int y) const {
    return planes + F.plane_off[k] + (size_t)y * F.g.pw[k];
  }
};

template <int MODE, bool ENC, typename PL, bool ONE = false, bool LUT = false>
__device__ __forceinline__ void color_rows(const DecFrame &F, const Geom &g, const PL &pl,
                                           uint8_t *__restrict__ pix, const EncFrame *__restrict__ efr, int y0, int x0,
                                           bool two, int bgr, int invert, const uint8_t *lut = nullptr) {
  const int y1 = two ? y0 + 1 : y0;
  int v0[3][8], v1[3][8];
  if constexpr (MODE == 0) {
    uint2 q[3][2];
#pragma unroll
    for (int k = 0; k < 3; ++k) {
      q[k][0] = *reinterpret_cast<const uint2 *>(pl.row(k, y0) + x0);
      q[k][1] = *reinterpret_cast<const uint2 *>(pl.row(k, y1) + x0);
    }
#pragma unroll
    for (int k = 0; k < 3; ++k) {
      unpack8(q[k][0], v0[k]);
      unpack8(q[k][1], v1[k]);
    }
  } else {
    const uint2 qa = *reinterpret_cast<const uint2 *>(pl.row(0, y0) + x0);
    const uint2 qb = *reinterpret_cast<const uint2 *>(pl.row(0, y1) + x0);
    const int dw = g.dw[1], dh = g.dh[1];
    const bool fancy = (F.flags & 1) && dw > 2;
    const int i0 = x0 >> 1;
    int ix[6];
#pragma unroll
    for (int m = 0; m < 6; ++m) ix[m] = min(max(i0 - 1 + m, 0), dw - 1);
    constexpr int NR = MODE == 2 ? 3 : 2;
    int rows[NR];
    if constexpr (MODE == 2) {
      const int iy = min(y0 >> 1, dh - 1);
      rows[0] = max(iy - 1, 0);
      rows[1] = iy;
      rows[2] = min(iy + 1, dh - 1);
    } else {
      rows[0] = min(y0, dh - 1);
      rows[1] = min(y1, dh - 1);
    }
    int b[2][NR][6];
    const int e = min(dw - 1 - i0, 3);
    int sh[4];
#pragma unroll
    for (int m = 0; m < 4; ++m) sh[m] = 8 * min(m, e);
#pragma unroll
    for (int k = 0; k < 2; ++k) {
#pragma unroll
      for (int rr = 0; rr < NR; ++rr) {
        const uint8_t *r = pl.row(k + 1, rows[rr]);
        const uint32_t mid = *reinterpret_cast<const uint32_t *>(r + i0);
        b[k][rr][0] = r[ix[0]];
#pragma unroll
        for (int m = 1; m < 5; ++m) b[k][rr][m] = (int)((mid >> sh[m - 1]) & 0xFF);
        b[k][rr][5] = r[ix[5]];
      }
    }
    unpack8(qa, v0[0]);
    unpack8(qb, v1[0]);
#pragma unroll
    for (int k = 0; k < 2; ++k) {
      int c0[6], c1[6];
#pragma unroll
      for (int m = 0; m < 6; ++m) {
        if constexpr (MODE == 2) {
          c0[m] = fancy ? 3 * b[k][1][m] + b[k][0][m] : b[k][1][m];
          c1[m] = fancy ? 3 * b[k][1][m] + b[k][2][m] : b[k][1][m];
        } else {
          c0[m] = b[k][0][m];
          c1[m] = b[k][1][m];
        }
      }
      up2(c0, i0, dw, fancy, MODE == 2 ? 2 : 1, v0[k + 1]);
      up2(c1, i0, dw, fancy, MODE == 2 ? 2 : 1, v1[k + 1]);
    }
  }
  if constexpr (ENC) {
    uint32_t p0[8], p1[8];
#pragma unroll
    for (int rw = 0; rw < (ONE ? 1 : 2); ++rw)
#pragma unroll
      for (int j = 0; j < 8; ++j) {
        const int yy = rw ? v1[0][j] : v0[0][j], cb = rw ? v1[1][j] : v0[1][j], cr = rw ? v1[2][j] : v0[2][j];
        const int xcr = cr - 128, xcb = cb - 128;
        const uint32_t r = clamp255(yy + ((__mul24(91881, xcr) + 32768) >> 16));
        const uint32_t gg = clamp255(yy + ((__mul24(-22554, xcb) + 32768 - __mul24(46802, xcr)) >> 16));
        const uint32_t b = clamp255(yy + ((__mul24(116130, xcb) + 32768) >> 16));
        uint32_t px;
        if constexpr (LUT) px = lut[512 + r] | (uint32_t)lut[256 + gg] << 8 | (uint32_t)lut[b] << 16;
        else px = (r | gg << 8 | b << 16) ^ (invert ? 0xFFFFFFu : 0u);
        if (rw) p1[j] = two ? px : p0[j];
        else p0[j] = px;
      }
    return enc_store_rows<ONE>(efr[blockIdx.z], pix, p0, p1, y0, x0, g.w);
  }
  uint8_t o0[24], o1[24];
  ycc8<LUT>(v0, 3, bgr, invert, o0, lut);
  ycc8<LUT>(v1, 3, bgr, invert, o1, lut);
  const int w = g.w;
  uint8_t *const d0 = pix + F.out_off + ((size_t)y0 * w + x0) * 3, *const d1 = d0 + (size_t)w * 3;
  store24(d0, w - x0, o0);
  if (two) store24(d1, w - x0, o1);
}

template <bool LUT>
struct ColorFilter {
  typedef int Arg;
  static __device__ __forceinline__ int invert(int f) { return f; }
};
template <>
struct ColorFilter<true> {
  typedef LutTable Arg;
  static __device__ __forceinline__ int invert(const LutTable &) { return 0; }
};

__device__ __forceinline__ void stage_lut(uint32_t *s_lut, const LutTable &tab) {
  if (threadIdx.x < 192) s_lut[threadIdx.x] = tab.w[threadIdx.x];
}

template <bool ENC, int CM, bool LUT = false>
__global__ __launch_bounds__(256) void k_color(const DecFrame *__restrict__ fr, const uint8_t *__restrict__ planes,
                                               uint8_t *__restrict__ pix, const EncFrame *__restrict__ efr, int bgr,
                                               const typename ColorFilter<LUT>::Arg filt) {
  const uint8_t *lut = nullptr;
  if constexpr (LUT) {
    __shared__ uint32_t s_lut[192];
    stage_lut(s_lut, filt);
    __syncthreads();
    lut = reinterpret_cast<const uint8_t *>(s_lut);
  }
  const int invert = ColorFilter<LUT>::invert(filt);
  const DecFrame &F = fr[blockIdx.z];
  const Geom &g = F.g;
  const int y0 = blockIdx.y * 2, x0 = (blockIdx.x * 256 + threadIdx.x) * 8;
  if (y0 >= g.h || x0 >= g.w) return;
  const bool two = y0 + 1 < g.h;
  const uint32_t cm = CM >= 0 ? (uint32_t)CM : (F.flags >> 1) & 3u;
  const GlobalPlanes gp{planes, F};
  if (cm == 1) return color_rows<0, ENC, GlobalPlanes, false, LUT>(F, g, gp, pix, efr, y0, x0, two, bgr, invert, lut);
  if (cm == 2) return color_rows<1, ENC, GlobalPlanes, false, LUT>(F, g, gp, pix, efr, y0, x0, two, bgr, invert, lut);
  if (cm == 3) return color_rows<2, ENC, GlobalPlanes, false, LUT>(F, g, gp, pix, efr, y0, x0, two, bgr, invert, lut);
  uint8_t o0[24], o1[24];
  color8<LUT>(F, g, planes, y0, x0, bgr, invert, o0, lut);
  color8<LUT>(F, g, planes, two ? y0 + 1 : y0, x0, bgr, invert, o1, lut);
  if constexpr (ENC) return enc_sample_rows(efr[blockIdx.z], pix, o0, o1, y0, x0, g.w, bgr);
  const int w = g.w;
  uint8_t *const d0 = pix + F.out_off + ((size_t)y0 * w + x0) * 3;
  store24(d0, w - x0, o0);
  if (two) store24(d0 + (size_t)w * 3, w - x0, o1);
}

constexpr int kStripMcus = 15;
constexpr int kStripY = kStripMcus * 16;
constexpr int kStripC = (kStripMcus + 2) * 8;

struct StripPlanes {
  const uint8_t *y, *cb, *cr;
  int y_base, x_base, c_base;
  __device__ __forceinline__ const uint8_t *row(int k, int yy) const {
    const int r = yy - y_base;
    return k == 0 ? y + r * kStripY - x_base : (k == 1 ? cb : cr) + r * kStripC - c_base;
  }
};

template <bool ONE, bool LUT = false>
__global__ __launch_bounds__(256) void k_idct_color422(const DecFrame *__restrict__ fr, const int16_t *coef,
                                                       const int32_t *dcseq, const uint8_t *nmask,
                                                       uint8_t *__restrict__ eplanes, const EncFrame *__restrict__ efr,
                                                       const typename ColorFilter<LUT>::Arg filt) {
  const DecFrame &F = fr[blockIdx.z];
  const Geom &g = F.g;
  const int mcux = g.mcux, my = blockIdx.y, m0 = blockIdx.x * kStripMcus;
  if (m0 >= mcux || my >= g.mcuy) return;
  __shared__ int32_t blkv[kIdctBlocks][72];
  __shared__ __attribute__((aligned(16))) uint16_t s_qz[3][64];
  __shared__ uint8_t s_pos[64];
  __shared__ uint32_t s_col[8];
  uint8_t *const s_y = reinterpret_cast<uint8_t *>(&blkv[0][0]);
  uint8_t *const s_cb = s_y + 8 * kStripY, *const s_cr = s_cb + 8 * kStripC;
  static_assert(8 * (kStripY + 2 * kStripC) <= (int)sizeof(blkv), "strip fits the coefficient rows");
  const uint32_t t = threadIdx.x, slot = t >> 3, r = t & 7;
  bool valid[kIdctNb];
  uint32_t kk[kIdctNb], lx[kIdctNb];
  uint4 raw[kIdctNb];
  int32_t dc[kIdctNb];
  uint32_t nm[kIdctNb];
#pragma unroll
  for (int h = 0; h < kIdctNb; ++h) {
    const int b = h * 32 + (int)slot;
    const int k = b < 30 ? 0 : b < 47 ? 1 : 2;
    const int j = k == 0 ? b : k == 1 ? b - 30 : b - 47;
    const int mx = k == 0 ? m0 + (j >> 1) : m0 - 1 + j;
    const int c = k == 0 ? (j & 1) : k + 1;
    kk[h] = (uint32_t)k;
    lx[h] = (uint32_t)j;
    valid[h] = mx >= 0 && mx < mcux;
    const uint64_t mcu = (uint64_t)my * mcux + (valid[h] ? mx : 0);
    const uint64_t bi = valid[h] ? F.blk0 + mcu * 4 + c : F.blk0;
    const uint64_t di = valid[h] ? F.dcbase[k] + mcu * (k == 0 ? 2 : 1) + (k == 0 ? (j & 1) : 0) : F.dcbase[0];
    raw[h] = *reinterpret_cast<const uint4 *>(coef + bi * 64 + r * 8);
    dc[h] = dcseq[di];
    nm[h] = nmask ? (uint32_t)nmask[bi] : 0xFFu;
  }
  if (t < 192) s_qz[t >> 6][kZigOf[t & 63]] = F.q[t >> 6][t & 63];
  if (t < 64) s_pos[t] = kIdctPos[t];
  if (t < 8) s_col[t] = kIdctCol[t];
  const uint8_t *lut = nullptr;
  if constexpr (LUT) {
    __shared__ uint32_t s_lut[192];
    stage_lut(s_lut, filt);
    lut = reinterpret_cast<const uint8_t *>(s_lut);
  }
  __syncthreads();
  const uint2 pos8 = *reinterpret_cast<const uint2 *>(&s_pos[r * 8]);
  const uint32_t colg = s_col[r];
#pragma unroll
  for (int h = 0; h < kIdctNb; ++h) {
    if (!valid[h]) continue;
    const bool st = (nm[h] >> r) & 1;
    const uint32_t qw[4] = {st ? raw[h].x : 0u, st ? raw[h].y : 0u, st ? raw[h].z : 0u, st ? raw[h].w : 0u};
    const uint4 q4 = *reinterpret_cast<const uint4 *>(&s_qz[kk[h]][r * 8]);
    const uint32_t qq[4] = {q4.x, q4.y, q4.z, q4.w};
#pragma unroll
    for (int j = 0; j < 8; ++j) {
      const int32_t v = (r == 0 && j == 0) ? (int32_t)(int16_t)dc[h] : (int32_t)(int16_t)(qw[j >> 1] >> (16 * (j & 1)));
      const uint32_t at = ((j < 4 ? pos8.x : pos8.y) >> (8 * (j & 3))) & 0xFF;
      blkv[h * 32 + slot][at] = __mul24(v, (int32_t)((qq[j >> 1] >> (16 * (j & 1))) & 0xFFFF));
    }
  }
  __syncthreads();
  int32_t col[kIdctNb][8];
  const auto pass1 = [&](auto m24) {
#pragma unroll
    for (int h = 0; h < kIdctNb; ++h) {
      if (!valid[h]) continue;
      int32_t in[8];
#pragma unroll
      for (int i = 0; i < 8; ++i) in[i] = blkv[h * 32 + slot][i * 8 + ((colg >> (4 * i)) & 7)];
      idct_line<decltype(m24)::value>(in, col[h], 11);
    }
  };
  if (F.flags & kDecIdct24) pass1(BoolTag<true>{});
  else pass1(BoolTag<false>{});
  __syncthreads();
#pragma unroll
  for (int h = 0; h < kIdctNb; ++h) {
    if (!valid[h]) continue;
#pragma unroll
    for (int i = 0; i < 8; ++i) blkv[h * 32 + slot][i * 9 + r] = col[h][i];
  }
  __syncthreads();
  uint2 row8[kIdctNb];
#pragma unroll
  for (int h = 0; h < kIdctNb; ++h) {
    int32_t in[8];
    uint32_t out[8];
#pragma unroll
    for (int i = 0; i < 8; ++i) in[i] = blkv[h * 32 + slot][r * 9 + i];
    idct_row_limited(in, out);
    uint32_t lo = 0, hi = 0;
#pragma unroll
    for (int i = 0; i < 4; ++i) {
      lo |= out[i] << (8 * i);
      hi |= out[i + 4] << (8 * i);
    }
    row8[h] = make_uint2(lo, hi);
  }
  __syncthreads();
#pragma unroll
  for (int h = 0; h < kIdctNb; ++h) {
    if (!valid[h]) continue;
    uint8_t *dst = kk[h] == 0 ? s_y + r * kStripY : (kk[h] == 1 ? s_cb : s_cr) + r * kStripC;
    *reinterpret_cast<uint2 *>(dst + lx[h] * 8) = row8[h];
  }
  __syncthreads();
  constexpr int kRows = ONE ? 1 : 2;
  if (t >= (uint32_t)(2 * kStripMcus * (8 / kRows))) return;
  const int px = (int)t % (2 * kStripMcus), rp = (int)t / (2 * kStripMcus);
  const int y0 = my * 8 + kRows * rp, x0 = m0 * 16 + px * 8;
  if (y0 >= g.h || x0 >= g.w) return;
  const StripPlanes sp{s_y, s_cb, s_cr, my * 8, m0 * 16, (m0 - 1) * 8};
  color_rows<1, true, StripPlanes, ONE, LUT>(F, g, sp, eplanes, efr, y0, x0, !ONE && y0 + 1 < g.h, 0,
                                             ColorFilter<LUT>::invert(filt), lut);
}


__device__ __forceinline__ int32_t m24(int32_t a, int32_t b) { return __mul24(a, b); }

__device__ __forceinline__ void fdct_islow_line(int32_t p[8], int pass) {
  int32_t tmp0 = p[0] + p[7], tmp7 = p[0] - p[7];
  int32_t tmp1 = p[1] + p[6], tmp6 = p[1] - p[6];
  int32_t tmp2 = p[2] + p[5], tmp5 = p[2] - p[5];
  int32_t tmp3 = p[3] + p[4], tmp4 = p[3] - p[4];
  const int32_t tmp10 = tmp0 + tmp3, tmp13 = tmp0 - tmp3;
  const int32_t tmp11 = tmp1 + tmp2, tmp12 = tmp1 - tmp2;
  const int sh = pass ? 15 : 11;
  const int32_t rnd = 1 << (sh - 1);
  if (!pass) {
    p[0] = (tmp10 + tmp11) * 4;
    p[4] = (tmp10 - tmp11) * 4;
  } else {
    p[0] = DESCALE(tmp10 + tmp11, 2);
    p[4] = DESCALE(tmp10 - tmp11, 2);
  }
  const int32_t z1 = m24(tmp12 + tmp13, FIX_0_541196100) + rnd;
  p[2] = (z1 + m24(tmp13, FIX_0_765366865)) >> sh;
  p[6] = (z1 + m24(tmp12, -FIX_1_847759065)) >> sh;
  const int32_t z5 = m24(tmp4 + tmp6 + tmp5 + tmp7, FIX_1_175875602) + rnd;
  const int32_t z1o = m24(tmp4 + tmp7, -FIX_0_899976223), z2 = m24(tmp5 + tmp6, -FIX_2_562915447);
  const int32_t z3 = m24(tmp4 + tmp6, -FIX_1_961570560) + z5, z4 = m24(tmp5 + tmp7, -FIX_0_390180644) + z5;
  p[7] = (m24(tmp4, FIX_0_298631336) + z1o + z3) >> sh;
  p[5] = (m24(tmp5, FIX_2_053119869) + z2 + z4) >> sh;
  p[3] = (m24(tmp6, FIX_3_072711026) + z2 + z3) >> sh;
  p[1] = (m24(tmp7, FIX_1_501321110) + z1o + z4) >> sh;
}

__device__ __forceinline__ void fdct_ifast_line(int32_t p[8]) {
  int32_t tmp0 = p[0] + p[7], tmp7 = p[0] - p[7];
  int32_t tmp1 = p[1] + p[6], tmp6 = p[1] - p[6];
  int32_t tmp2 = p[2] + p[5], tmp5 = p[2] - p[5];
  int32_t tmp3 = p[3] + p[4], tmp4 = p[3] - p[4];
  int32_t tmp10 = tmp0 + tmp3, tmp13 = tmp0 - tmp3;
  int32_t tmp11 = tmp1 + tmp2, tmp12 = tmp1 - tmp2;
  p[0] = tmp10 + tmp11;
  p[4] = tmp10 - tmp11;
  const int32_t z1 = m24(tmp12 + tmp13, 181) >> 8;
  p[2] = tmp13 + z1;
  p[6] = tmp13 - z1;
  tmp10 = tmp4 + tmp5;
  tmp11 = tmp5 + tmp6;
  tmp12 = tmp6 + tmp7;
  const int32_t z5 = m24(tmp10 - tmp12, 98) >> 8;
  const int32_t z2 = (m24(tmp10, 139) >> 8) + z5;
  const int32_t z4 = (m24(tmp12, 334) >> 8) + z5;
  const int32_t z3 = m24(tmp11, 181) >> 8;
  const int32_t z11 = tmp7 + z3, z13 = tmp7 - z3;
  p[5] = z13 + z2;
  p[3] = z13 - z2;
  p[1] = z11 + z4;
  p[7] = z11 - z4;
}

__device__ __forceinline__ int16_t quantize(int32_t x, uint32_t recip, uint32_t corr, uint32_t sh) {
  const int32_t t = (int16_t)x;
  const int32_t sg = t >> 31;
  const uint32_t a = (uint32_t)((t ^ sg) - sg);
  const uint32_t p = ((a + corr) * recip) >> (sh & 31);
  return (int16_t)(((int32_t)p ^ sg) - sg);
}

static_assert(kAcScratchWords % 4 == 0 && kAcScratchWords / 4 <= 16, "two 16-B stores per lane");
__device__ __forceinline__ void clear_ac_words(uint32_t *acw_slot, uint32_t r) {
  uint4 *a4 = reinterpret_cast<uint4 *>(acw_slot);
  a4[r] = make_uint4(0, 0, 0, 0);
  if (r + 8 < (uint32_t)kAcScratchWords / 4) a4[r + 8] = make_uint4(0, 0, 0, 0);
}

template <int H, int R>
struct RowPix {
  uint32_t wd[R][6 * H];
  const uint8_t *row[R];
  bool fast;
};
template <int H, int R>
__device__ __forceinline__ void rows_load(const uint8_t *img, int w, int h, int px, int py, bool real,
                                          const uint8_t *dummy, RowPix<H, R> &p) {
  p.fast = real && px + 8 * H <= w;
#pragma unroll
  for (int y = 0; y < R; ++y) {
    p.row[y] = img + (size_t)min(py + y, h - 1) * w * 3;
    p.fast = p.fast && ((reinterpret_cast<uintptr_t>(p.row[y]) + (uintptr_t)px * 3) & 3) == 0;
  }
#pragma unroll
  for (int y = 0; y < R; ++y) {
    const uint32_t *s32 = reinterpret_cast<const uint32_t *>(p.fast ? p.row[y] + (size_t)px * 3 : dummy);
#pragma unroll
    for (int i = 0; i < 6 * H; ++i) p.wd[y][i] = s32[i];
  }
}

template <int H, int R>
__device__ __forceinline__ void rows_conv(const RowPix<H, R> &p, int w, int px, const Ycc &q, int32_t v[8]) {
#pragma unroll
  for (int j = 0; j < 8; ++j) v[j] = 0;
  if (p.fast) {
#pragma unroll
    for (int y = 0; y < R; ++y)
#pragma unroll
      for (int x = 0; x < 8 * H; ++x) {
        const int c0 = (int)((p.wd[y][(3 * x) / 4] >> (8 * ((3 * x) % 4))) & 0xFF);
        const int c1 = (int)((p.wd[y][(3 * x + 1) / 4] >> (8 * ((3 * x + 1) % 4))) & 0xFF);
        const int c2 = (int)((p.wd[y][(3 * x + 2) / 4] >> (8 * ((3 * x + 2) % 4))) & 0xFF);
        v[x / H] += ycc_apply(q, c0, c1, c2);
      }
  } else {
#pragma unroll
    for (int y = 0; y < R; ++y)
#pragma unroll
      for (int x = 0; x < 8 * H; ++x) {
        const uint8_t *b = p.row[y] + (size_t)min(px + x, w - 1) * 3;
        v[x / H] += ycc_apply(q, b[0], b[1], b[2]);
      }
  }
}

template <int H, int R, bool FAST>
__device__ __forceinline__ void fdct_pass1(const uint8_t *img, const Geom &g, int bx, int sy, Ycc q, bool real,
                                           const uint4 &tw, const uint8_t *dummy, uint4 *s_tab, uint32_t *acw_slot,
                                           uint32_t r, int32_t *wsrow) {
  RowPix<H, R> p;
  const int px = bx * 8 * H;
  rows_load<H, R>(img, g.w, g.h, px, sy * R, real, dummy, p);
  if (threadIdx.x < 192) s_tab[threadIdx.x] = tw;
  clear_ac_words(acw_slot, r);
  if (!real) return;
  if (H == 1 && R == 1) q.bias -= 128 << 16;
  int32_t v[8];
  rows_conv<H, R>(p, g.w, px, q, v);
#pragma unroll
  for (int j = 0; j < 8; ++j) {
    if (H == 2 && R == 1) v[j] = (v[j] + (j & 1) - 256) >> 1;
    if (H == 2 && R == 2) v[j] = (v[j] + 1 + (j & 1) - 512) >> 2;
    if (H == 1 && R == 2) v[j] = (v[j] + 1 - 256) >> 1;
  }
  if (FAST) fdct_ifast_line(v);
  else fdct_islow_line(v, 0);
#pragma unroll
  for (int j = 0; j < 8; ++j) wsrow[j] = v[j];
}

#ifndef VF_ABL
#define VF_ABL 0
#endif
template <bool FAST>
__device__ __forceinline__ void fdct_pass1_planes(const uint8_t *plane, int pitch, int bx, int sy, bool real,
                                                  const uint4 &tw, const uint8_t *dummy, uint4 *s_tab,
                                                  uint32_t *acw_slot, uint32_t r, int32_t *wsrow) {
#if VF_ABL & 1
  const uint2 q = make_uint2((uint32_t)(bx * 0x01010101) ^ (uint32_t)sy, (uint32_t)(sy * 0x01030507) ^ r);
#else
  const uint2 q = *reinterpret_cast<const uint2 *>(real ? plane + (size_t)sy * pitch + bx * 8 : dummy);
#endif
  if (threadIdx.x < 192) s_tab[threadIdx.x] = tw;
  clear_ac_words(acw_slot, r);
  if (!real) return;
  int32_t v[8];
#pragma unroll
  for (int j = 0; j < 8; ++j) v[j] = (int32_t)(((j < 4 ? q.x : q.y) >> (8 * (j & 3))) & 0xFF) - 128;
#if !(VF_ABL & 2)
  if (FAST) fdct_ifast_line(v);
  else fdct_islow_line(v, 0);
#endif
#pragma unroll
  for (int j = 0; j < 8; ++j) wsrow[j] = v[j];
}

constexpr uint32_t kAcWords = kAcScratchWords;

__device__ __forceinline__ uint64_t acs_idx(uint64_t gb, uint32_t i) {
  return (gb >> 6) * (64ull * kAcWords) + (uint64_t)i * 64 + (gb & 63);
}

struct LdsBits {
  uint32_t *w;
  uint32_t wi, n;
  uint64_t acc;
  __device__ __forceinline__ LdsBits(uint32_t *words, uint32_t pos) : w(words), wi(pos >> 5), n(pos & 31), acc(0) {}
  __device__ __forceinline__ void put(uint32_t bits, uint32_t size) {
    acc = (acc << size) | bits;
    n += size;
    const bool full = n >= 32;
    const uint32_t lo = (uint32_t)acc, hi = (uint32_t)(acc >> 32);
    atomicOr(w + wi, __builtin_amdgcn_alignbit(full ? hi : lo, full ? lo : 0u, n & 31));
    wi += full ? 1u : 0u;
    n &= 31;
  }
  __device__ __forceinline__ void finish() {
    atomicOr(w + wi, __builtin_amdgcn_alignbit((uint32_t)acc, 0u, n));
  }
};

__device__ __forceinline__ uint32_t or8(uint32_t x) {
  x |= (uint32_t)__builtin_amdgcn_mov_dpp((int)x, 0xB1, 0xF, 0xF, false);
  x |= (uint32_t)__builtin_amdgcn_mov_dpp((int)x, 0x4E, 0xF, 0xF, false);
  x |= (uint32_t)__builtin_amdgcn_mov_dpp((int)x, 0x141, 0xF, 0xF, false);
  return x;
}
__device__ __forceinline__ uint32_t scan8(uint32_t x, uint32_t r) {
  uint32_t y = (uint32_t)__builtin_amdgcn_mov_dpp((int)x, 0x111, 0xF, 0xF, false);
  x += r >= 1 ? y : 0u;
  y = (uint32_t)__builtin_amdgcn_mov_dpp((int)x, 0x112, 0xF, 0xF, false);
  x += r >= 2 ? y : 0u;
  y = (uint32_t)__builtin_amdgcn_mov_dpp((int)x, 0x114, 0xF, 0xF, false);
  x += r >= 4 ? y : 0u;
  return x;
}
__device__ __forceinline__ uint32_t last8(uint32_t x) {
  return (uint32_t)__builtin_amdgcn_ds_swizzle((int)x, 0xF8);
}


__device__ __forceinline__ uint32_t qo_at(uint32_t slot, uint32_t zz) {
  return zz ^ (((0x7250u >> (4 * (slot & 3))) & 7) << 3);
}

constexpr uint32_t kFdctGroup = 8;
template <int CH, int CV, bool FAST, bool PL>
__global__ __launch_bounds__(256) __attribute__((amdgpu_waves_per_eu(8))) void k_fdct(const EncFrame *__restrict__ fr, const EncTables *tab, const uint8_t *pix,
                                              int16_t *dcq, uint32_t *acbits, uint32_t *acscr, int bgr) {
  const EncFrame &F = fr[blockIdx.y];
  const Geom &g = F.g;
  const uint32_t bpm = (uint32_t)g.bpm, nmcu = (uint32_t)g.nmcu;
  const uint32_t ngroups = (nmcu + kFdctGroup - 1) / kFdctGroup;
  if (blockIdx.x * 4 >= ngroups * bpm) return;
  __shared__ int32_t ws[32][8][9];
  __shared__ __attribute__((aligned(16))) uint32_t acw[32][kAcWords];
  __shared__ uint4 s_tab[192];
#if VF_ABL & 16
  const uint4 tw = make_uint4(threadIdx.x, 0x3F3F3F3Fu, threadIdx.x, 0x3F3F3F3Fu);
#else
  const uint4 tw = threadIdx.x < 192 ? reinterpret_cast<const uint4 *>(tab->fdct_lds)[threadIdx.x] : make_uint4(0, 0, 0, 0);
#endif
  const uint2 (*const s_q)[64] = reinterpret_cast<const uint2 (*)[64]>(s_tab);
  const uint32_t (*const s_ac)[256] = reinterpret_cast<const uint32_t (*)[256]>(reinterpret_cast<const uint32_t *>(s_tab) + 256);
  const uint32_t slot = threadIdx.x >> 3, r = threadIdx.x & 7, lm = slot & (kFdctGroup - 1);
  int16_t *const qo = reinterpret_cast<int16_t *>(&ws[slot][0][0]);
  const uint32_t unit = blockIdx.x * 4 + __builtin_amdgcn_readfirstlane(threadIdx.x >> 6);
  const uint32_t grp = unit / bpm, c = unit - grp * bpm;
  const uint32_t mcu = grp * kFdctGroup + lm;
  const uint32_t b = mcu * bpm + c;
  uint32_t k = 0, bx = 0, by = 0;
  bool real = false;
  if (grp < ngroups) {
    k = (uint32_t)g.bcomp[c];
    const uint32_t mcux = (uint32_t)g.mcux;
    uint32_t mx = (grp * kFdctGroup) % mcux + lm, my = (grp * kFdctGroup) / mcux;
    while (mx >= mcux) mx -= mcux, ++my;
    bx = mx * (uint32_t)g.mh[k] + (uint32_t)g.bxo[c];
    by = my * (uint32_t)g.mv[k] + (uint32_t)g.byo[c];
    real = mcu < nmcu && bx < (uint32_t)g.wb[k] && by < (uint32_t)g.hb[k];
  }
  const uint8_t *img = pix + F.img_off;
  const uint8_t *dummy = reinterpret_cast<const uint8_t *>(tab->fdct_lds);
  {
    const int sy = min((int)(by * 8 + r), (int)g.rrows[k] - 1);
    if constexpr (PL) {
      fdct_pass1_planes<FAST>(pix + F.eplane_off[k], g.wb[k] * 8, (int)bx, sy, real, tw, dummy, s_tab, acw[slot], r,
                              ws[slot][r]);
    } else {
      const Ycc q = ycc_coefs((int)k, bgr != 0);
      if (k == 0) fdct_pass1<1, 1, FAST>(img, g, (int)bx, sy, q, real, tw, dummy, s_tab, acw[slot], r, ws[slot][r]);
      else fdct_pass1<CH, CV, FAST>(img, g, (int)bx, sy, q, real, tw, dummy, s_tab, acw[slot], r, ws[slot][r]);
    }
  }
  __syncthreads();
  const int t = k > 0;
  if (real) {
    int32_t v[8];
#pragma unroll
    for (int i = 0; i < 8; ++i) v[i] = ws[slot][i][r];
#if !(VF_ABL & 2)
    if (FAST) fdct_ifast_line(v);
    else fdct_islow_line(v, 1);
#endif
    const uint32_t qsel = 8 + 6 * (slot & 3);
#pragma unroll
    for (int i = 0; i < 8; ++i) {
      const uint2 q = s_q[t][i * 8 + r];
#if VF_ABL & 32
      qo[(q.y >> qsel) & 63] = (int16_t)(v[i] >> 3);
#else
      qo[(q.y >> qsel) & 63] = quantize(v[i], q.x & 0xFFFF, q.x >> 16, q.y);
#endif
    }
  }
  __builtin_amdgcn_fence(__ATOMIC_SEQ_CST, "wavefront");
  int vz[8];
  {
    const uint4 q4 = real ? *reinterpret_cast<const uint4 *>(&qo[qo_at(slot, r * 8)]) : make_uint4(0, 0, 0, 0);
    const uint32_t qw[4] = {q4.x, q4.y, q4.z, q4.w};
#pragma unroll
    for (int j = 0; j < 8; ++j) vz[j] = (int)(int16_t)(qw[j >> 1] >> (16 * (j & 1)));
  }
  uint32_t m8 = 0;
#pragma unroll
  for (int j = 0; j < 8; ++j)
    if (vz[j] != 0 && (r | j) != 0) m8 |= 1u << j;
  const uint64_t mask = ((uint64_t)or8(r < 4 ? 0u : m8 << (8 * (r - 4))) << 32) | or8(r < 4 ? m8 << (8 * r) : 0u);
  const uint32_t zrl = s_ac[t][0xF0], eobc = s_ac[t][0x00];
  const uint32_t zlen = zrl & 0xFF;
  const bool eob = mask == 0 || (63 - __clzll(mask)) < 63;
  int prev = r ? 63 - __clzll((mask | 1ull) & ((1ull << (8 * r)) - 1)) : 0;
#if VF_ABL & 64
  if (m8 != 12345u) {
    if (real && r == 0) {
      dcq[F.blk0 + b] = (int16_t)vz[0];
      acbits[F.blk0 + b] = eob ? 2u : 3u;
    }
    return;
  }
#endif
  const uint32_t cnt = __popc(m8);
  const uint32_t rinc = scan8(cnt, r);
  const uint32_t nnz = last8(rinc);
  uint32_t *const lst = reinterpret_cast<uint32_t *>(&ws[slot][0][0]);
  {
    uint32_t *wp = lst + (rinc - cnt);
    uint32_t *const spare = lst + 64 + r;
#pragma unroll
    for (int j = 0; j < 8; ++j) {
      const int kk = 8 * (int)r + j;
      const bool nz = (m8 >> j) & 1;
      *(nz ? wp : spare) = ((uint32_t)(kk - prev - 1) << 16) | (uint32_t)(uint16_t)vz[j];
      wp += nz ? 1 : 0;
      prev = nz ? kk : prev;
    }
  }
  __builtin_amdgcn_fence(__ATOMIC_SEQ_CST, "wavefront");
  uint32_t off = 0;
#if VF_ABL & 4
  if (nnz != 12345) {
    if (real && r == 0) {
      dcq[F.blk0 + b] = (int16_t)vz[0];
      acbits[F.blk0 + b] = 2u;
    }
    return;
  }
#endif
  for (uint32_t q0 = 0; __ballot(q0 < nnz) != 0; q0 += 8) {
    const uint32_t q = q0 + r;
    const bool act = q < nnz;
    const uint32_t ent = act ? lst[q] : 0u;
    const uint32_t run = ent >> 16;
    const int v = (int)(int16_t)(ent & 0xFFFF);
    const uint32_t av = (uint32_t)(v < 0 ? -v : v);
    const uint32_t nb = 32 - __clz(av);
    const uint32_t e = s_ac[t][((run & 15) << 4) + (nb & 15)];
    const uint32_t code = ((e >> 8) << nb) | ((uint32_t)(v < 0 ? v - 1 : v) & ((1u << nb) - 1));
    const uint32_t clen = (e & 0xFF) + nb;
    const uint32_t nzr = run >> 4;
    const uint32_t nbits = act ? __umul24(nzr, zlen) + clen : 0u;
    const uint32_t incl = scan8(nbits, r);
    if (act) {
      LdsBits out(acw[slot], off + incl - nbits);
      for (uint32_t z = nzr; z; --z) out.put(zrl >> 8, zlen);
      out.put(code, clen);
      out.finish();
    }
    off += last8(incl);
  }
  if (real && eob && r == 0) {
    LdsBits out(acw[slot], off);
    out.put(eobc >> 8, eobc & 0xFF);
    out.finish();
  }
  const uint32_t total = off + (eob ? (eobc & 0xFF) : 0u);
  __builtin_amdgcn_fence(__ATOMIC_SEQ_CST, "wavefront");
  if (real) {
    const uint64_t gb = F.blk0 + b;
    const uint32_t nw = (total + 31) >> 5;
    for (uint32_t i = r; i < nw; i += 8) acscr[acs_idx(gb, i)] = acw[slot][i];
    if (r == 0) {
      dcq[gb] = (int16_t)vz[0];
      acbits[gb] = total;
    }
  }
}


__device__ __forceinline__ uint32_t wire_mask(uint32_t a, uint32_t b) {
  const uint32_t m = (0xFFFFFFFFu >> a) & (b >= 32 ? 0xFFFFFFFFu : ~(0xFFFFFFFFu >> b));
  return bswap32(m);
}
__device__ __forceinline__ void merge_word(uint32_t *w, uint32_t mask, uint32_t v) {
  atomicAnd(w, ~mask);
  atomicOr(w, v);
}

struct BitSink {
  uint32_t *w;
  uint32_t wi;
  uint64_t acc;
  uint32_t n, s;
  bool first;
  __device__ __forceinline__ BitSink(uint32_t *words, uint32_t off)
      : w(words), wi(off >> 5), acc(0), n(off & 31), s(off & 31), first(true) {}
  __device__ __forceinline__ void put(uint32_t code, uint32_t size) {
    acc = (acc << size) | code;
    n += size;
    if (n >= 32) {
      n -= 32;
      const uint32_t v = (uint32_t)(acc >> n);
      if (first) merge_word(w + wi, wire_mask(s, 32), bswap32(v));
      else w[wi] = bswap32(v);
      first = false;
      ++wi;
      acc &= n ? ((1ull << n) - 1) : 0ull;
    }
  }
  __device__ __forceinline__ void finish() {
    if (n) merge_word(w + wi, wire_mask(first ? s : 0u, n), bswap32((uint32_t)(acc << (32 - n))));
  }
};

__device__ __forceinline__ uint32_t dc_category(int diff) {
  const uint32_t a = (uint32_t)(diff < 0 ? -diff : diff);
  return a ? 32 - __clz(a) : 0;
}

constexpr uint32_t kDummyAc = 0x80000000u;
__device__ __forceinline__ int enc_dc_at(const Geom &g, const int16_t *dcq, int mx, int my, int xi, int yi, int mh,
                                         int mv, int wb, int hb, int cf) {
  for (;;) {
    const int bx = mx * mh + xi, by = my * mv + yi;
    if (by >= hb) {
      yi -= 1;
      xi = mh - 1;
      continue;
    }
    if (bx >= wb) {
      xi -= 1;
      continue;
    }
    return dcq[((uint64_t)my * (uint32_t)g.mcux + (uint32_t)mx) * (uint32_t)g.bpm + (uint32_t)(cf + yi * mh + xi)];
  }
}

__global__ __launch_bounds__(256) void k_len(const EncFrame *__restrict__ fr, const EncTables *tab, const int16_t *dcq,
                                             uint32_t *acbits, uint32_t *bits, uint32_t *pre) {
  const EncFrame &F = fr[blockIdx.y];
  const Geom &g = F.g;
  const uint32_t bpm = (uint32_t)g.bpm, nmcu = (uint32_t)g.nmcu, mcux = (uint32_t)g.mcux;
  const uint32_t ngroups = (nmcu + 63) / 64;
  const uint32_t unit = blockIdx.x * 4 + __builtin_amdgcn_readfirstlane(threadIdx.x >> 6);
  if (unit >= ngroups * bpm) return;
  const uint32_t grp = unit / bpm, c = unit - grp * bpm;
  const uint32_t mcu = grp * 64 + (threadIdx.x & 63);
  if (mcu >= nmcu) return;
  const int k = g.bcomp[c], mh = g.mh[k], mv = g.mv[k], wb = g.wb[k], hb = g.hb[k], cf = g.cfirst[k];
  int mx = (int)((grp * 64) % mcux + (threadIdx.x & 63)), my = (int)((grp * 64) / mcux);
  while (mx >= (int)mcux) mx -= (int)mcux, ++my;
  const int dc = enc_dc_at(g, dcq + F.blk0, mx, my, g.bxo[c], g.byo[c], mh, mv, wb, hb, cf);
  int pred = 0;
  if ((int)c > cf) {
    pred = enc_dc_at(g, dcq + F.blk0, mx, my, g.bxo[c - 1], g.byo[c - 1], mh, mv, wb, hb, cf);
  } else if (mcu > 0) {
    const int pmx = mx > 0 ? mx - 1 : (int)mcux - 1, pmy = mx > 0 ? my : my - 1;
    pred = enc_dc_at(g, dcq + F.blk0, pmx, pmy, mh - 1, mv - 1, mh, mv, wb, hb, cf);
  }
  const bool dummy = mx * mh + g.bxo[c] >= wb || my * mv + g.byo[c] >= hb;
  const int diff = dc - pred;
  const int t = k > 0;
  const uint32_t nb = dc_category(diff);
  const uint32_t e = tab->dc[t][nb];
  const uint32_t extra = nb ? ((uint32_t)(diff < 0 ? diff - 1 : diff) & ((1u << nb) - 1)) : 0u;
  const uint64_t gb = F.blk0 + (uint64_t)mcu * bpm + c;
  pre[gb] = ((((e >> 8) << nb) | extra) << 5) | ((e & 0xFF) + nb);
  uint32_t ac;
  if (dummy) {
    const uint32_t eob = tab->ac[t][0];
    acbits[gb] = kDummyAc | ((eob >> 8) << 5) | (eob & 0xFF);
    ac = eob & 0xFF;
  } else {
    ac = acbits[gb];
  }
  bits[gb] = (e & 0xFF) + nb + ac;
}

struct LdsSink {
  uint32_t *w;
  uint32_t wi;
  uint64_t acc;
  uint32_t n;
  __device__ __forceinline__ LdsSink(uint32_t *words, uint32_t off) : w(words), wi(off >> 5), acc(0), n(off & 31) {}
  __device__ __forceinline__ void put(uint32_t code, uint32_t size) {
    acc = (acc << size) | code;
    n += size;
    if (n >= 32) {
      n -= 32;
      atomicOr(w + wi, bswap32((uint32_t)(acc >> n)));
      ++wi;
      acc &= n ? ((1ull << n) - 1) : 0ull;
    }
  }
  __device__ __forceinline__ void finish() {
    if (n) atomicOr(w + wi, bswap32((uint32_t)(acc << (32 - n))));
  }
};

template <typename Sink>
__device__ __forceinline__ void pack_block(Sink &out, uint32_t p, uint32_t n, uint32_t a0, const uint32_t *aw) {
  out.put(p >> 5, p & 31);
  if (n & kDummyAc) {
    out.put((n & ~kDummyAc) >> 5, n & 31);
  } else if (n) {
    if (n >= 32) {
      out.put(a0, 32);
      for (uint32_t i = 1; i < (n >> 5); ++i) out.put(aw[64 * i], 32);
      if (n & 31) out.put(aw[64 * (n >> 5)] >> (32 - (n & 31)), n & 31);
    } else {
      out.put(a0 >> (32 - n), n);
    }
  }
  out.finish();
}

constexpr uint32_t kPackWords = 1024;
__global__ __launch_bounds__(256) void k_pack(const EncFrame *__restrict__ fr, const uint32_t *pre, const uint32_t *acbits,
                                              const uint32_t *acscr, const uint32_t *bitoff, uint8_t *stream) {
  __shared__ uint32_t s_img[4][kPackWords];
  const EncFrame &F = fr[blockIdx.y];
  const uint32_t nblocks = (uint32_t)F.g.nblocks, lane = threadIdx.x & 63, wv = threadIdx.x >> 6;
  const uint32_t bw0 = blockIdx.x * 256 + wv * 64;
  if (bw0 >= nblocks) return;
  const uint32_t last = min(63u, nblocks - 1 - bw0), b = bw0 + lane;
  const bool valid = lane <= last;
  const uint64_t gb = F.blk0 + (valid ? b : bw0);
  const uint32_t p = pre[gb], n = acbits[gb], off = bitoff[gb];
  const uint32_t *aw = acscr + acs_idx(gb, 0);
  const uint32_t a0 = aw[0];
  uint32_t *words = reinterpret_cast<uint32_t *>(stream + F.bits_off);
  const uint32_t len = (p & 31) + ((n & kDummyAc) ? (n & 31) : n);
  const uint32_t w0 = __shfl(off, 0) >> 5, w1 = (__shfl(off + len, (int)last) + 31) >> 5;
  const uint32_t nw = w1 - w0;
  if (nw > kPackWords) {
    if (valid) {
      BitSink out(words, off);
      pack_block(out, p, n, a0, aw);
    }
    return;
  }
  uint32_t *img = s_img[wv];
  for (uint32_t i = lane; i < nw; i += 64) img[i] = 0;
  __builtin_amdgcn_fence(__ATOMIC_RELEASE, "wavefront");
  __builtin_amdgcn_wave_barrier();
  __builtin_amdgcn_fence(__ATOMIC_ACQUIRE, "wavefront");
  if (valid) {
    LdsSink out(img, off - w0 * 32);
    pack_block(out, p, n, a0, aw);
  }
  __builtin_amdgcn_fence(__ATOMIC_RELEASE, "wavefront");
  __builtin_amdgcn_wave_barrier();
  __builtin_amdgcn_fence(__ATOMIC_ACQUIRE, "wavefront");
  const uint32_t s0 = __shfl(off, 0) & 31, e1 = __shfl(off + len, (int)last) - (w1 - 1) * 32;
  for (uint32_t i = lane; i < nw; i += 64) {
    const uint32_t v = img[i];
    if (i == 0 || i == nw - 1) merge_word(words + w0 + i, wire_mask(i == 0 ? s0 : 0u, i == nw - 1 ? e1 : 32u), v);
    else words[w0 + i] = v;
  }
}


__device__ __forceinline__ uint32_t ff_bytes(const uint8_t *s, uint32_t nbytes, uint32_t tb, uint32_t i0,
                                             uint8_t *bytes) {
  const uint4 q = *reinterpret_cast<const uint4 *>(s + i0);
  const uint32_t qw[4] = {q.x, q.y, q.z, q.w};
  uint32_t n = 0;
#pragma unroll
  for (int j = 0; j < 16; ++j) {
    const uint32_t i = i0 + j;
    uint8_t v = i < nbytes ? (uint8_t)(qw[j >> 2] >> (8 * (j & 3))) : 0;
    if (i == nbytes - 1 && (tb & 7)) v |= (uint8_t)(0xFF >> (tb & 7));
    bytes[j] = v;
    n += (i < nbytes && v == 0xFF);
  }
  return n;
}

__global__ __launch_bounds__(256) void k_ff_count(const EncFrame *__restrict__ fr, const uint32_t *total_bits,
                                                  const uint8_t *stream, uint32_t *cnt) {
  const uint32_t ntiles_max = fr[blockIdx.y].ntiles_max, tile0 = fr[blockIdx.y].tile0;
  const uint8_t *src = stream + fr[blockIdx.y].bits_off;
  __shared__ uint32_t sh[4];
  const uint32_t tb = total_bits[blockIdx.y], nbytes = (tb + 7) >> 3;
  for (uint32_t t = blockIdx.x; t < ntiles_max; t += gridDim.x) {
    if (t * kTile < nbytes) {
      uint8_t bytes[16];
      const uint32_t i0 = t * kTile + threadIdx.x * 16;
      const uint32_t n = i0 < nbytes ? ff_bytes(src, nbytes, tb, i0, bytes) : 0;
      uint32_t tot;
      (void)wg_excl_scan(n, sh, &tot);
      if (threadIdx.x == 0) cnt[tile0 + t] = tot;
      __syncthreads();
    } else if (threadIdx.x == 0) {
      cnt[tile0 + t] = 0;
    }
  }
}

__global__ __launch_bounds__(256) void k_ff_write(const EncFrame *__restrict__ fr, const uint32_t *total_bits,
                                                  const uint8_t *stream, const uint32_t *off, const uint32_t *nff,
                                                  const uint8_t *hdr, uint8_t *pack, uint64_t *out_size) {
  const EncFrame &F = fr[blockIdx.y];
  const uint32_t hdr_len = F.hdr_len, hdr_off = F.hdr_off, tile0 = F.tile0;
  const uint8_t *src = stream + F.bits_off;
  const uint32_t tb = total_bits[blockIdx.y], nbytes = (tb + 7) >> 3;
  const uint32_t ntiles = (nbytes + kTile - 1) / kTile;
  __shared__ uint32_t sh[4];
  __shared__ uint64_t s_pack;
  if (threadIdx.x < 64) {
    uint64_t acc = 0;
    for (uint32_t g = threadIdx.x; g < blockIdx.y; g += 64)
      acc += ((uint64_t)fr[g].hdr_len + ((total_bits[g] + 7) >> 3) + nff[g] + 2 + 63) & ~63ull;
#pragma unroll
    for (int o = 32; o > 0; o >>= 1) acc += __shfl_xor(acc, o, 64);
    if (threadIdx.x == 0) s_pack = acc;
  }
  __syncthreads();
  uint8_t *o = pack + s_pack;
  __shared__ uint8_t s_out[2 * kTile];
  for (uint32_t t = blockIdx.x; t < ntiles; t += gridDim.x) {
    if (t == 0)
      for (uint32_t j = threadIdx.x; j < hdr_len; j += 256) o[j] = hdr[hdr_off + j];
    uint8_t bytes[16];
    const uint32_t i0 = t * kTile + threadIdx.x * 16;
    const uint32_t n = i0 < nbytes ? ff_bytes(src, nbytes, tb, i0, bytes) : 0;
    uint32_t tot;
    uint32_t lp = threadIdx.x * 16 + wg_excl_scan(n, sh, &tot);
    for (int j = 0; j < 16; ++j) {
      if (i0 + j >= nbytes) break;
      s_out[lp++] = bytes[j];
      if (bytes[j] == 0xFF) s_out[lp++] = 0;
    }
    __syncthreads();
    const uint32_t len = min((uint32_t)kTile, nbytes - t * kTile) + tot;
    uint8_t *dst = o + (uint64_t)hdr_len + t * kTile + off[tile0 + t];
    const uint32_t head = min((uint32_t)(-(uintptr_t)dst & 3), len), nw = (len - head) >> 2;
    if (threadIdx.x < head) dst[threadIdx.x] = s_out[threadIdx.x];
    for (uint32_t i = threadIdx.x; i < nw; i += 256) {
      const uint32_t a = head + 4 * i;
      reinterpret_cast<uint32_t *>(dst + head)[i] = (uint32_t)s_out[a] | ((uint32_t)s_out[a + 1] << 8) |
                                                    ((uint32_t)s_out[a + 2] << 16) | ((uint32_t)s_out[a + 3] << 24);
    }
    const uint32_t tail = head + 4 * nw;
    if (threadIdx.x < len - tail) dst[tail + threadIdx.x] = s_out[tail + threadIdx.x];
    if (t == ntiles - 1 && threadIdx.x == 0) {
      const uint64_t size = (uint64_t)hdr_len + nbytes + nff[blockIdx.y] + 2;
      o[size - 2] = 0xFF;
      o[size - 1] = 0xD9;
      out_size[blockIdx.y] = size;
    }
    __syncthreads();
  }
}

}


hipError_t scan_u32(const ScanSeg *segs, int nseg, uint32_t max_tiles, const uint32_t *in, uint32_t *out,
                    uint32_t *tsum, uint32_t *totals, bool inclusive, hipStream_t s) {
  return seg_scan<uint32_t>(segs, nseg, max_tiles, in, out, tsum, totals, inclusive, s);
}

hipError_t scan_i32(const ScanSeg *segs, int nseg, uint32_t max_tiles, const int32_t *in, int32_t *out,
                    int32_t *tsum, int32_t *totals, bool inclusive, hipStream_t s) {
  return seg_scan<int32_t>(segs, nseg, max_tiles, in, out, tsum, totals, inclusive, s);
}

hipError_t dec_unstuff_count(const DecSeg *__restrict__ sg, int nseg, uint32_t max_tiles, const uint8_t *in, uint32_t *tile_cnt,
                             hipStream_t s) {
  if (nseg <= 0 || !max_tiles) return hipSuccess;
  hipLaunchKernelGGL(k_unstuff_count, dim3(max_tiles, (unsigned)nseg), dim3(256), 0, s, sg, in, tile_cnt);
  return hipGetLastError();
}

hipError_t dec_unstuff_write(const DecSeg *__restrict__ sg, int nseg, uint32_t max_tiles, const uint8_t *in,
                             const uint32_t *tile_off, const uint32_t *us_len, uint8_t *us, hipStream_t s) {
  if (nseg <= 0 || !max_tiles) return hipSuccess;
  hipLaunchKernelGGL(k_unstuff_write, dim3(max_tiles, (unsigned)nseg), dim3(256), 0, s, sg, in, tile_off, us_len, us);
  return hipGetLastError();
}

hipError_t dec_sync(const DecSeg *__restrict__ sg, const DecFrame *__restrict__ fr, int nseg, uint32_t max_sub, const uint8_t *us,
                    const uint32_t *us_len, const uint64_t *exit_in, uint64_t *exit_out, const uint32_t *cnt_in,
                    uint32_t *cnt_out, uint64_t *used, uint64_t *ck, uint32_t *ckrem, uint32_t *changed, int pass,
                    hipStream_t s) {
  if (nseg <= 0 || !max_sub) return hipSuccess;
  hipLaunchKernelGGL(k_sync, dim3((max_sub + 255) / 256, (unsigned)nseg), dim3(256), 0, s, sg, fr, us, us_len,
                     exit_in, exit_out, cnt_in, cnt_out, used, ck, ckrem, changed, pass);
  return hipGetLastError();
}

hipError_t dec_syncg(int G, const DecSeg *__restrict__ sg, const DecFrame *__restrict__ fr, int nseg, uint32_t max_sub,
                     const uint8_t *us, const uint32_t *us_len, uint64_t *exits, uint32_t *cnts, uint64_t *used,
                     uint64_t *ck, uint32_t *ckrem, uint32_t *changed, int pass, uint32_t warm, int tabs4,
                     hipStream_t s) {
  if (nseg <= 0 || !max_sub) return hipSuccess;
  warm = std::min<uint32_t>(warm, kSyncWarmMax) & ~31u;
#define VF_SYNCG(GG, ND, LS)                                                                                      \
  if (G == GG && (ND == 2) == (tabs4 != 0) && LS == (tabs4 == 2)) {                                               \
    const uint32_t span = syncg_threads(GG) * GG;                                                                 \
    hipLaunchKernelGGL((k_syncg<GG, ND, LS>), dim3((max_sub + span - 1) / span, (unsigned)nseg),                  \
                       dim3(syncg_threads(GG)), 0, s, sg, fr, us, us_len, exits, cnts, used, ck, ckrem, changed,  \
                       pass, warm);                                                                               \
    return hipGetLastError();                                                                                     \
  }
  VF_SYNCG(1, 3, false)
  VF_SYNCG(2, 3, false)
  VF_SYNCG(3, 3, false)
  VF_SYNCG(4, 3, false)
  VF_SYNCG(8, 3, false)
  VF_SYNCG(4, 2, false)
  VF_SYNCG(5, 2, false)
  VF_SYNCG(4, 2, true)
  VF_SYNCG(5, 2, true)
#undef VF_SYNCG
  return hipErrorInvalidValue;
}

hipError_t dec_sync_spec(const DecSeg *__restrict__ sg, const DecFrame *__restrict__ fr, int nseg, uint32_t max_wg, const uint8_t *us,
                         const uint32_t *us_len, const SpecBufs &b, uint64_t *exit_out, uint32_t *cnt_out,
                         uint32_t *unresolved, int lsb, hipStream_t s) {
  if (nseg <= 0 || !max_wg) return hipSuccess;
  if (lsb) hipLaunchKernelGGL(k_spec<true>, dim3(max_wg, (unsigned)nseg), dim3(256), 0, s, sg, fr, us, us_len, b);
  else hipLaunchKernelGGL(k_spec<false>, dim3(max_wg, (unsigned)nseg), dim3(256), 0, s, sg, fr, us, us_len, b);
  hipLaunchKernelGGL(k_resolve, dim3((unsigned)nseg), dim3(256), 0, s, sg, fr, us, us_len, b, unresolved);
  hipLaunchKernelGGL(k_finalize, dim3(max_wg, (unsigned)nseg), dim3(256), 0, s, sg, fr, us_len, b, exit_out, cnt_out);
  return hipGetLastError();
}

hipError_t dec_write(const DecSeg *__restrict__ sg, const DecFrame *__restrict__ fr, int nseg, uint32_t max_sub, const uint8_t *us,
                     const uint32_t *us_len, const uint64_t *exits, const uint32_t *bstart, int16_t *coef,
                     int32_t *dcseq, uint8_t *nmask, hipStream_t s) {
  if (nseg <= 0 || !max_sub) return hipSuccess;
  const dim3 grid((max_sub + 255) / 256, (unsigned)nseg);
  if (nmask)
    hipLaunchKernelGGL(k_write<true>, grid, dim3(256), 0, s, sg, fr, us, us_len, exits, bstart, coef, dcseq, nmask);
  else
    hipLaunchKernelGGL(k_write<false>, grid, dim3(256), 0, s, sg, fr, us, us_len, exits, bstart, coef, dcseq, nmask);
  return hipGetLastError();
}

hipError_t dec_write4(const DecSeg *__restrict__ sg, const DecFrame *__restrict__ fr, int nseg, uint32_t max_sub, const uint8_t *us,
                      const uint32_t *us_len, const uint64_t *exits, const uint32_t *cnt, const uint64_t *ck,
                      const uint32_t *ckrem, const uint32_t *bstart, int16_t *coef, int32_t *dcseq, uint8_t *nmask,
                      hipStream_t s) {
  if (nseg <= 0 || !max_sub) return hipSuccess;
  const dim3 grid((max_sub + 63) / 64, (unsigned)nseg);
  if (nmask)
    hipLaunchKernelGGL(k_write4<true>, grid, dim3(256), 0, s, sg, fr, us, us_len, exits, cnt, ck, ckrem, bstart, coef,
                       dcseq, nmask);
  else
    hipLaunchKernelGGL(k_write4<false>, grid, dim3(256), 0, s, sg, fr, us, us_len, exits, cnt, ck, ckrem, bstart, coef,
                       dcseq, nmask);
  return hipGetLastError();
}

hipError_t dec_idct(const DecFrame *__restrict__ fr, int n, uint32_t max_blocks, const int16_t *coef, const int32_t *dcseq,
                    const uint8_t *nmask, uint8_t *planes, hipStream_t s) {
  if (n <= 0 || !max_blocks) return hipSuccess;
  hipLaunchKernelGGL(k_idct, dim3((max_blocks + 150 + 63) / 64, (unsigned)n), dim3(256), 0, s, fr,
                     coef, dcseq, nmask, planes);
  return hipGetLastError();
}

hipError_t dec_color(const DecFrame *__restrict__ fr, int n, int max_w, int max_h, const uint8_t *planes, uint8_t *pix, int bgr,
                     int invert, const EncFrame *efr, int cm, hipStream_t s, const LutTable *lut) {
  if (n <= 0 || max_w <= 0 || max_h <= 0) return hipSuccess;
  const dim3 grid((unsigned)((max_w + 2047) / 2048), (unsigned)((max_h + 1) / 2), (unsigned)n);
#define VF_COLOR(E, C)                                                                                    \
  do {                                                                                                    \
    if (lut) hipLaunchKernelGGL((k_color<E, C, true>), grid, dim3(256), 0, s, fr, planes, pix, efr, bgr, *lut); \
    else hipLaunchKernelGGL((k_color<E, C>), grid, dim3(256), 0, s, fr, planes, pix, efr, bgr, invert);  \
  } while (0)
  if (efr) {
    if (cm == 0) VF_COLOR(true, 0);
    else if (cm == 1) VF_COLOR(true, 1);
    else if (cm == 2) VF_COLOR(true, 2);
    else if (cm == 3) VF_COLOR(true, 3);
    else VF_COLOR(true, -1);
  } else {
    if (cm == 0) VF_COLOR(false, 0);
    else if (cm == 1) VF_COLOR(false, 1);
    else if (cm == 2) VF_COLOR(false, 2);
    else if (cm == 3) VF_COLOR(false, 3);
    else VF_COLOR(false, -1);
  }
#undef VF_COLOR
  return hipGetLastError();
}

hipError_t dec_idct_color422(const DecFrame *__restrict__ fr, int n, int max_w, int max_h, const int16_t *coef,
                             const int32_t *dcseq, const uint8_t *nmask, uint8_t *eplanes, const EncFrame *efr,
                             int invert, int one_row, hipStream_t s, const LutTable *lut) {
  if (n <= 0 || max_w <= 0 || max_h <= 0) return hipSuccess;
  const unsigned mcux = (unsigned)((max_w + 15) / 16), mcuy = (unsigned)((max_h + 7) / 8);
  const dim3 grid((mcux + kStripMcus - 1) / kStripMcus, mcuy, (unsigned)n);
  if (lut && one_row)
    hipLaunchKernelGGL((k_idct_color422<true, true>), grid, dim3(256), 0, s, fr, coef, dcseq, nmask, eplanes, efr, *lut);
  else if (lut)
    hipLaunchKernelGGL((k_idct_color422<false, true>), grid, dim3(256), 0, s, fr, coef, dcseq, nmask, eplanes, efr, *lut);
  else if (one_row)
    hipLaunchKernelGGL(k_idct_color422<true>, grid, dim3(256), 0, s, fr, coef, dcseq, nmask, eplanes, efr, invert);
  else
    hipLaunchKernelGGL(k_idct_color422<false>, grid, dim3(256), 0, s, fr, coef, dcseq, nmask, eplanes, efr, invert);
  return hipGetLastError();
}

hipError_t enc_fdct(const EncFrame *__restrict__ fr, int n, uint32_t max_blocks, const EncTables *tab, const uint8_t *pix,
                    int16_t *dcq, uint32_t *acbits, uint32_t *acscr, int bgr, int fastdct, int ch, int cv, int planes,
                    hipStream_t s) {
  if (n <= 0 || !max_blocks) return hipSuccess;
  const dim3 grid((max_blocks + 70 + 31) / 32, (unsigned)n);
  if (planes) {
    if (fastdct) hipLaunchKernelGGL((k_fdct<1, 1, true, true>), grid, dim3(256), 0, s, fr, tab, pix, dcq, acbits, acscr, bgr);
    else hipLaunchKernelGGL((k_fdct<1, 1, false, true>), grid, dim3(256), 0, s, fr, tab, pix, dcq, acbits, acscr, bgr);
    return hipGetLastError();
  }
#define VF_FDCT(CH, CV)                                                                                              \
  if (ch == CH && cv == CV) {                                                                                        \
    if (fastdct)                                                                                                     \
      hipLaunchKernelGGL((k_fdct<CH, CV, true, false>), grid, dim3(256), 0, s, fr, tab, pix, dcq, acbits, acscr, bgr); \
    else                                                                                                             \
      hipLaunchKernelGGL((k_fdct<CH, CV, false, false>), grid, dim3(256), 0, s, fr, tab, pix, dcq, acbits, acscr, bgr); \
    return hipGetLastError();                                                                                        \
  }
  VF_FDCT(1, 1)
  VF_FDCT(2, 1)
  VF_FDCT(2, 2)
  VF_FDCT(1, 2)
#undef VF_FDCT
  return hipErrorInvalidValue;
}

hipError_t enc_len(const EncFrame *__restrict__ fr, int n, uint32_t max_blocks, const EncTables *tab, const int16_t *dcq,
                   uint32_t *acbits, uint32_t *bits, uint32_t *pre, hipStream_t s) {
  if (n <= 0 || !max_blocks) return hipSuccess;
  hipLaunchKernelGGL(k_len, dim3((max_blocks / 64 + 10 + 3) / 4, (unsigned)n), dim3(256), 0, s, fr, tab, dcq, acbits,
                     bits, pre);
  return hipGetLastError();
}

hipError_t enc_pack(const EncFrame *__restrict__ fr, int n, uint32_t max_blocks, const uint32_t *pre, const uint32_t *acbits,
                    const uint32_t *acscr, const uint32_t *bitoff, const uint32_t *total_bits, uint8_t *stream,
                    hipStream_t s) {
  if (n <= 0 || !max_blocks) return hipSuccess;
  hipLaunchKernelGGL(k_pack, dim3((max_blocks + 255) / 256, (unsigned)n), dim3(256), 0, s, fr, pre, acbits, acscr,
                     bitoff, stream);
  return hipGetLastError();
}

constexpr uint32_t kFFGrid = 64;

hipError_t enc_ff_count(const EncFrame *__restrict__ fr, int n, uint32_t max_tiles, const uint32_t *total_bits,
                        const uint8_t *stream, uint32_t *tile_cnt, hipStream_t s) {
  if (n <= 0 || !max_tiles) return hipSuccess;
  hipLaunchKernelGGL(k_ff_count, dim3(max_tiles < kFFGrid ? max_tiles : kFFGrid, (unsigned)n), dim3(256), 0, s, fr,
                     total_bits, stream, tile_cnt);
  return hipGetLastError();
}

hipError_t enc_ff_write(const EncFrame *__restrict__ fr, int n, uint32_t max_tiles, const uint32_t *total_bits,
                        const uint8_t *stream, const uint32_t *tile_off, const uint32_t *nff, const uint8_t *hdr,
                        uint8_t *pack, uint64_t *out_size, hipStream_t s) {
  if (n <= 0 || !max_tiles) return hipSuccess;
  hipLaunchKernelGGL(k_ff_write, dim3(max_tiles < kFFGrid ? max_tiles : kFFGrid, (unsigned)n), dim3(256), 0, s, fr,
                     total_bits, stream, tile_off, nff, hdr, pack, out_size);
  return hipGetLastError();
}

}
}
```

### distributed-video-filter_amd/csrc/vf_jpeg_plan.h

```cpp
#pragma once
#include <algorithm>
#include <cstdint>
#include <cstdlib>
#include <cstring>

#include "vf_env.h"
#include "vf_jpeg_types.h"

namespace vf {
namespace jpeg {

struct JpegSwitches {
  const char *sync = nullptr;
  const char *sync_lsb = nullptr;
  const char *sync_tabs4 = nullptr;
  const char *sync_g = nullptr;
  const char *sync_queued = nullptr;
  const char *sync_warm = nullptr;
  const char *sync_stats = nullptr;
  const char *chunks = nullptr;
  const char *write4 = nullptr;
  const char *fuse = nullptr;
  const char *fuse_idct = nullptr;
  const char *idct24 = nullptr;
  const char *fetch_learn = nullptr;
  const char *trace = nullptr;

  static JpegSwitches read() {
    JpegSwitches s;
    s.sync = env_str("VF_JPEG_SYNC");
    s.sync_lsb = env_str("VF_JPEG_SYNC_LSB");
    s.sync_tabs4 = env_str("VF_JPEG_SYNC_TABS4");
    s.sync_g = env_str("VF_JPEG_SYNC_G");
    s.sync_queued = env_str("VF_JPEG_SYNC_QUEUED");
    s.sync_warm = env_str("VF_JPEG_SYNC_WARM");
    s.sync_stats = env_str("VF_JPEG_SYNC_STATS");
    s.chunks = env_str("VF_JPEG_CHUNKS");
    s.write4 = env_str("VF_JPEG_WRITE4");
    s.fuse = env_str("VF_JPEG_FUSE");
    s.fuse_idct = env_str("VF_JPEG_FUSE_IDCT");
    s.idct24 = env_str("VF_JPEG_IDCT24");
    s.fetch_learn = env_str("VF_JPEG_FETCH_LEARN");
    s.trace = env_str("VF_JPEG_TRACE");
    return s;
  }
};

struct BatchTraits {
  bool spec_ok = true;
  bool tabs4 = true;
  bool pow2bpm = true;
  bool d422 = true;
  uint32_t max_sub = 0;
  uint64_t bits_per_block = 0;
};

struct DecodePlan {
  bool spec = false;
  int g = 4;
  int tabs = 0;
  int queued = kQueuedPasses;
  uint32_t warm = 0;
  bool lsb = false;
  bool chunks = false;
  bool write4 = true;
  bool fuse = false;
  bool fuse_idct = false;
  bool enc_fast = false;
  bool stats = false;
  bool trace = false;
};

inline DecodePlan resolve(const JpegSwitches &sw, const BatchTraits &t, bool fuse_requested) {
  DecodePlan p;
  constexpr uint32_t kSpecAutoSubs = 12288;
  const bool force_pass = sw.sync && std::strcmp(sw.sync, "pass") == 0;
  const bool force_spec = sw.sync && std::strcmp(sw.sync, "spec") == 0;
  p.spec = t.spec_ok && !force_pass && (force_spec || t.max_sub <= kSpecAutoSubs);
  p.lsb = t.pow2bpm && flag_on(sw.sync_lsb);
  const bool t4 = t.tabs4 && flag_on(sw.sync_tabs4);
  const int g = sw.sync_g ? std::atoi(sw.sync_g) : 5;
  p.g = g == 5 ? (t4 ? 5 : 4) : (g >= 0 && g <= 4) || g == 8 ? g : 4;
  p.tabs = t4 && (p.g == 4 || p.g == 5) ? (p.lsb ? 2 : 1) : 0;
  p.queued = sw.sync_queued ? std::min(std::max(std::atoi(sw.sync_queued), 1), kQueuedPasses) : kQueuedPasses;
  if (sw.sync_warm && *sw.sync_warm && std::strcmp(sw.sync_warm, "auto") != 0)
    p.warm = (uint32_t)std::strtoul(sw.sync_warm, nullptr, 10);
  else
    p.warm = (uint32_t)std::min<uint64_t>(4096, 12 * t.bits_per_block) & ~31u;
  constexpr uint64_t kChunkBitsPerBlock = 128;
  p.chunks = sw.chunks && *sw.chunks ? std::strcmp(sw.chunks, "0") != 0
                                     : p.spec || t.bits_per_block <= kChunkBitsPerBlock;
  p.write4 = flag_on(sw.write4);
  p.fuse = fuse_requested && flag_on(sw.fuse);
  p.fuse_idct = p.fuse && t.d422 && flag_on(sw.fuse_idct);
  p.stats = sw.sync_stats != nullptr;
  p.trace = sw.trace != nullptr;
  return p;
}

}
}
```

Before: 513,700 frames/s.

## Add fixed-geometry 4:2:2 paths for fused IDCT-color store and FDCT

Adds a specialised STD template path for 4:2:2-to-4:2:2 JPEG transcode. The fused IDCT/color kernel writes Y and horizontally downsampled Cb/Cr planes directly with hardcoded geometry, and the FDCT uses a 2D grid indexed by MCU row and column instead of generic division-based unit mapping. It is gated behind the VF_JPEG_STD422 env flag plus the fuse flags. It also adds many VF_ABL ablation hooks. The measured workload is the raw invert stream kernel, which this JPEG path likely does not touch.

After: 506,900 frames/s. -1.3%, worse.

```diff
diff --git a/distributed-video-filter_amd/csrc/vf_jpeg.h b/distributed-video-filter_amd/csrc/vf_jpeg.h
--- a/distributed-video-filter_amd/csrc/vf_jpeg.h
+++ b/distributed-video-filter_amd/csrc/vf_jpeg.h
@@ -61,11 +61,13 @@
                              const int32_t *dcseq, const uint8_t *nmask, uint8_t *eplanes, const EncFrame *efr,
                              int invert, int one_row,
                              hipStream_t s,
-                             const LutTable *lut = nullptr);
+                             const LutTable *lut = nullptr,
+                             int std422 = 0);
 
 hipError_t enc_fdct(const EncFrame *fr, int n, uint32_t max_blocks, const EncTables *tab, const uint8_t *pix,
                     int16_t *dcq, uint32_t *acbits, uint32_t *acscr, int bgr, int fastdct, int ch, int cv, int planes,
-                    hipStream_t s);
+                    hipStream_t s,
+                    int std_w = 0, int std_h = 0);
 hipError_t enc_len(const EncFrame *fr, int n, uint32_t max_blocks, const EncTables *tab, const int16_t *dcq,
                    uint32_t *acbits, uint32_t *bits, uint32_t *pre, hipStream_t s);
 hipError_t enc_pack(const EncFrame *fr, int n, uint32_t max_blocks, const uint32_t *pre, const uint32_t *acbits,
diff --git a/distributed-video-filter_amd/csrc/vf_jpeg_codec.h b/distributed-video-filter_amd/csrc/vf_jpeg_codec.h
--- a/distributed-video-filter_amd/csrc/vf_jpeg_codec.h
+++ b/distributed-video-filter_amd/csrc/vf_jpeg_codec.h
@@ -122,7 +122,8 @@
  private:
   int init(std::string *err);
   int prepare_decode(const uint8_t *const *jpegs, const size_t *sizes, int n, int flags, const JpegSwitches &sw,
-                     std::string *err);
+                     std::string *err,
+                     int enc_subsamp = -1);
   int run_decode(int bgr, std::string *err);
   int run_decode_post(int bgr, std::string *err);
   hipError_t span_pass(int p);
diff --git a/distributed-video-filter_amd/csrc/vf_jpeg_host.hip b/distributed-video-filter_amd/csrc/vf_jpeg_host.hip
--- a/distributed-video-filter_amd/csrc/vf_jpeg_host.hip
+++ b/distributed-video-filter_amd/csrc/vf_jpeg_host.hip
@@ -254,7 +254,7 @@
 }
 
 int Codec::prepare_decode(const uint8_t *const *jpegs, const size_t *sizes, int n, int flags, const JpegSwitches &sw,
-                          std::string *err) {
+                          std::string *err, int enc_subsamp) {
   if (n <= 0) {
     *err = "empty batch";
     return kInvalid;
@@ -513,6 +513,7 @@
     prep_ms_[2] = ms(tp2, clk::now());
   }
   traits.max_sub = dmax_sub_;
+  traits.e422 = enc_subsamp == 1;
   plan_ = resolve(sw, traits, filter_.in_colour());
   plan_.enc_fast = (flags & kFlagFastDct) != 0;
   return kOk;
@@ -651,7 +652,7 @@
     CK(stage_event(4));
     CK(dec_idct_color422(fr, n, dmax_w_, dmax_h_, d_coef_.as<int16_t>(), d_dcpred_.as<int32_t>(), nmask,
                          d_eplanes_.as<uint8_t>(), d_efr_.as<EncFrame>(), invert ? 1 : 0, kSampV[esub_] == 1 ? 1 : 0,
-                         s_, lut));
+                         s_, lut, pl.std422 ? 1 : 0));
     CK(stage_event(5));
     return kOk;
   }
@@ -833,7 +834,7 @@
   CK(stage_event(6));
   CK(enc_fdct(fr, n, emax_blocks_, tab, fuse ? d_eplanes_.as<uint8_t>() : pix, d_dcq_.as<int16_t>(),
               d_acbits_.as<uint32_t>(), d_acscr_.as<uint32_t>(), bgr, fastdct ? 1 : 0, kSampH[esub_], kSampV[esub_],
-              fuse ? 1 : 0, s_));
+              fuse ? 1 : 0, s_, plan_.std422 ? dmax_w_ : 0, plan_.std422 ? dmax_h_ : 0));
   CK(enc_len(fr, n, emax_blocks_, tab, d_dcq_.as<int16_t>(), d_acbits_.as<uint32_t>(), d_bits_.as<uint32_t>(),
              d_pre_.as<uint32_t>(), s_));
   uint32_t *total_bits = d_etotals_.as<uint32_t>();
@@ -1004,7 +1005,7 @@
   const JpegSwitches sw = JpegSwitches::read();
   using clk = std::chrono::steady_clock;
   const auto t0 = clk::now();
-  if ((rc = prepare_decode(jpegs, jsizes, n, flags, sw, err))) return rc;
+  if ((rc = prepare_decode(jpegs, jsizes, n, flags, sw, err, subsamp))) return rc;
   const auto t1 = clk::now();
   std::vector<int> ws((size_t)n), hs((size_t)n);
   std::vector<uint64_t> offs((size_t)n);
@@ -1139,7 +1140,7 @@
     return kInvalid;
   }
   filter_ = filter;
-  if ((rc = prepare_decode(jpegs, jsizes, n, flags, JpegSwitches::read(), err))) return rc;
+  if ((rc = prepare_decode(jpegs, jsizes, n, flags, JpegSwitches::read(), err, subsamp))) return rc;
   std::vector<int> ws((size_t)n), hs((size_t)n);
   std::vector<uint64_t> offs((size_t)n);
   for (int f = 0; f < n; ++f) {
diff --git a/distributed-video-filter_amd/csrc/vf_jpeg_kernels.hip b/distributed-video-filter_amd/csrc/vf_jpeg_kernels.hip
--- a/distributed-video-filter_amd/csrc/vf_jpeg_kernels.hip
+++ b/distributed-video-filter_amd/csrc/vf_jpeg_kernels.hip
@@ -1869,9 +1869,14 @@
   return __builtin_amdgcn_sdot2(pr, q.c, __mul24((int)((px >> q.sh) & 0xFF), q.m) + q.bias, false) >> 16;
 }
 
-template <bool ONE = false>
+#ifndef VF_ABL
+#define VF_ABL 0
+#endif
+
+template <bool ONE = false, bool STD = false>
 __device__ __forceinline__ void enc_store_rows(const EncFrame &E, uint8_t *__restrict__ eplanes, uint32_t (&p0)[8],
                                                uint32_t (&p1)[8], int y0, int x0, int w) {
+  static_assert(ONE || !STD, "4:2:2 output has no vertical downsampling");
   const Geom &ge = E.g;
   const bool edge = x0 + 8 >= w;
   uint32_t l0 = 0, l1 = 0;
@@ -1887,6 +1892,61 @@
       p0[p] = p > lp ? l0 : p0[p];
       p1[p] = p > lp ? l1 : p1[p];
     }
+  }
+  if constexpr (STD) {
+    {
+      const EncCoef q = enc_coef(0);
+      const int pitch = ((w + 7) >> 3) * 8;
+      uint8_t *const row = eplanes + E.eplane_off[0] + (size_t)y0 * pitch;
+      int c0[8];
+#pragma unroll
+      for (int p = 0; p < 8; ++p) c0[p] = enc_sample(p0[p], q);
+      uint32_t lo = 0, hi = 0;
+#if VF_ABL & 0x10000
+      lo = p0[0] ^ p0[1] ^ p0[2] ^ p0[3], hi = p0[4] ^ p0[5] ^ p0[6] ^ p0[7];
+#else
+#pragma unroll
+      for (int p = 0; p < 4; ++p) {
+        lo |= (uint32_t)c0[p] << (8 * p);
+        hi |= (uint32_t)c0[p + 4] << (8 * p);
+      }
+#endif
+#if VF_ABL & 8
+      if (lo == 0x12345678u && hi == 0x9ABCDEF0u)
+#endif
+      *reinterpret_cast<uint2 *>(row + x0) = make_uint2(lo, hi);
+      if (edge) {
+        const int ev = enc_sample(l0, q);
+        #pragma clang loop unroll(disable) vectorize(disable)
+        for (int xs = x0 + 8; xs < pitch; ++xs) row[xs] = (uint8_t)ev;
+      }
+    }
+    const int pitch = ((w + 15) >> 4) * 8;
+#pragma unroll 1
+    for (int k = 1; k < 3; ++k) {
+      const EncCoef q = enc_coef(k);
+      uint8_t *const row = eplanes + E.eplane_off[k] + (size_t)y0 * pitch;
+      int c0[8];
+#pragma unroll
+      for (int p = 0; p < 8; ++p) c0[p] = enc_sample(p0[p], q);
+      uint32_t v = 0;
+#if VF_ABL & 0x10000
+      v = (p0[0] ^ p0[1] ^ p0[2] ^ p0[3] ^ p0[4] ^ p0[5] ^ p0[6] ^ p0[7]) + (uint32_t)k;
+#else
+#pragma unroll
+      for (int i = 0; i < 4; ++i) v |= (uint32_t)((c0[2 * i] + c0[2 * i + 1] + (i & 1)) >> 1) << (8 * i);
+#endif
+#if VF_ABL & 8
+      if (v == 0x12345678u)
+#endif
+      *reinterpret_cast<uint32_t *>(row + (x0 >> 1)) = v;
+      if (edge) {
+        const int ev = enc_sample(l0, q);
+        #pragma clang loop unroll(disable) vectorize(disable)
+        for (int xs = (x0 + 8) >> 1; xs < pitch; ++xs) row[xs] = (uint8_t)ev;
+      }
+    }
+    return;
   }
 #pragma unroll 1
   for (int k = 0; k < ge.ncomp; ++k) {
@@ -2000,7 +2060,7 @@
   }
 };
 
-template <int MODE, bool ENC, typename PL, bool ONE = false, bool LUT = false>
+template <int MODE, bool ENC, typename PL, bool ONE = false, bool LUT = false, bool STD = false>
 __device__ __forceinline__ void color_rows(const DecFrame &F, const Geom &g, const PL &pl,
                                            uint8_t *__restrict__ pix, const EncFrame *__restrict__ efr, int y0, int x0,
                                            bool two, int bgr, int invert, const uint8_t *lut = nullptr) {
@@ -2070,8 +2130,13 @@
           c1[m] = b[k][1][m];
         }
       }
+#if VF_ABL & 0x4000
+#pragma unroll
+      for (int j = 0; j < 8; ++j) v0[k + 1][j] = c0[1 + (j >> 1)] ^ c0[5 * (j & 1)], v1[k + 1][j] = c1[1 + (j >> 1)] ^ c1[5 * (j & 1)];
+#else
       up2(c0, i0, dw, fancy, MODE == 2 ? 2 : 1, v0[k + 1]);
       up2(c1, i0, dw, fancy, MODE == 2 ? 2 : 1, v1[k + 1]);
+#endif
     }
   }
   if constexpr (ENC) {
@@ -2088,10 +2153,13 @@
         uint32_t px;
         if constexpr (LUT) px = lut[512 + r] | (uint32_t)lut[256 + gg] << 8 | (uint32_t)lut[b] << 16;
         else px = (r | gg << 8 | b << 16) ^ (invert ? 0xFFFFFFu : 0u);
+#if VF_ABL & 0x8000
+        px = (uint32_t)yy | (uint32_t)cb << 8 | (uint32_t)cr << 16;
+#endif
         if (rw) p1[j] = two ? px : p0[j];
         else p0[j] = px;
       }
-    return enc_store_rows<ONE>(efr[blockIdx.z], pix, p0, p1, y0, x0, g.w);
+    return enc_store_rows<ONE, STD>(efr[blockIdx.z], pix, p0, p1, y0, x0, g.w);
   }
   uint8_t o0[24], o1[24];
   ycc8<LUT>(v0, 3, bgr, invert, o0, lut);
@@ -2162,7 +2230,7 @@
   }
 };
 
-template <bool ONE, bool LUT = false>
+template <bool ONE, bool LUT = false, bool STD = false>
 __global__ __launch_bounds__(256) void k_idct_color422(const DecFrame *__restrict__ fr, const int16_t *coef,
                                                        const int32_t *dcseq, const uint8_t *nmask,
                                                        uint8_t *__restrict__ eplanes, const EncFrame *__restrict__ efr,
@@ -2197,9 +2265,15 @@
     const uint64_t mcu = (uint64_t)my * mcux + (valid[h] ? mx : 0);
     const uint64_t bi = valid[h] ? F.blk0 + mcu * 4 + c : F.blk0;
     const uint64_t di = valid[h] ? F.dcbase[k] + mcu * (k == 0 ? 2 : 1) + (k == 0 ? (j & 1) : 0) : F.dcbase[0];
+#if VF_ABL & 0x100
+    raw[h] = make_uint4((uint32_t)bi ^ t, (uint32_t)di * 0x00010003u, t * 0x00050007u, (uint32_t)bi + r);
+    dc[h] = (int32_t)(di & 0xFF);
+    nm[h] = 0xFFu;
+#else
     raw[h] = *reinterpret_cast<const uint4 *>(coef + bi * 64 + r * 8);
     dc[h] = dcseq[di];
     nm[h] = nmask ? (uint32_t)nmask[bi] : 0xFFu;
+#endif
   }
   if (t < 192) s_qz[t >> 6][kZigOf[t & 63]] = F.q[t >> 6][t & 63];
   if (t < 64) s_pos[t] = kIdctPos[t];
@@ -2213,6 +2287,7 @@
   __syncthreads();
   const uint2 pos8 = *reinterpret_cast<const uint2 *>(&s_pos[r * 8]);
   const uint32_t colg = s_col[r];
+#if !(VF_ABL & 0x200)
 #pragma unroll
   for (int h = 0; h < kIdctNb; ++h) {
     if (!valid[h]) continue;
@@ -2227,6 +2302,7 @@
       blkv[h * 32 + slot][at] = __mul24(v, (int32_t)((qq[j >> 1] >> (16 * (j & 1))) & 0xFFFF));
     }
   }
+#endif
   __syncthreads();
   int32_t col[kIdctNb][8];
   const auto pass1 = [&](auto m24) {
@@ -2236,18 +2312,28 @@
       int32_t in[8];
 #pragma unroll
       for (int i = 0; i < 8; ++i) in[i] = blkv[h * 32 + slot][i * 8 + ((colg >> (4 * i)) & 7)];
+#if VF_ABL & 0x200
+      in[0] ^= (int32_t)(raw[h].x ^ raw[h].y ^ raw[h].z ^ raw[h].w ^ (uint32_t)dc[h] ^ nm[h] ^ pos8.x ^ pos8.y);
+#endif
+#if VF_ABL & 0x400
+#pragma unroll
+      for (int i = 0; i < 8; ++i) col[h][i] = in[i];
+#else
       idct_line<decltype(m24)::value>(in, col[h], 11);
+#endif
     }
   };
   if (F.flags & kDecIdct24) pass1(BoolTag<true>{});
   else pass1(BoolTag<false>{});
   __syncthreads();
+#if !(VF_ABL & 0x800)
 #pragma unroll
   for (int h = 0; h < kIdctNb; ++h) {
     if (!valid[h]) continue;
 #pragma unroll
     for (int i = 0; i < 8; ++i) blkv[h * 32 + slot][i * 9 + r] = col[h][i];
   }
+#endif
   __syncthreads();
   uint2 row8[kIdctNb];
 #pragma unroll
@@ -2255,8 +2341,17 @@
     int32_t in[8];
     uint32_t out[8];
 #pragma unroll
+#if VF_ABL & 0x800
+    for (int i = 0; i < 8; ++i) in[i] = col[h][i];
+#else
     for (int i = 0; i < 8; ++i) in[i] = blkv[h * 32 + slot][r * 9 + i];
+#endif
+#if VF_ABL & 0x1000
+#pragma unroll
+    for (int i = 0; i < 8; ++i) out[i] = (uint32_t)in[i] & 0xFF;
+#else
     idct_row_limited(in, out);
+#endif
     uint32_t lo = 0, hi = 0;
 #pragma unroll
     for (int i = 0; i < 4; ++i) {
@@ -2270,6 +2365,9 @@
   for (int h = 0; h < kIdctNb; ++h) {
     if (!valid[h]) continue;
     uint8_t *dst = kk[h] == 0 ? s_y + r * kStripY : (kk[h] == 1 ? s_cb : s_cr) + r * kStripC;
+#if VF_ABL & 0x2000
+    if (row8[h].x == 0x12345678u && row8[h].y == 0x9ABCDEF0u)
+#endif
     *reinterpret_cast<uint2 *>(dst + lx[h] * 8) = row8[h];
   }
   __syncthreads();
@@ -2279,8 +2377,8 @@
   const int y0 = my * 8 + kRows * rp, x0 = m0 * 16 + px * 8;
   if (y0 >= g.h || x0 >= g.w) return;
   const StripPlanes sp{s_y, s_cb, s_cr, my * 8, m0 * 16, (m0 - 1) * 8};
-  color_rows<1, true, StripPlanes, ONE, LUT>(F, g, sp, eplanes, efr, y0, x0, !ONE && y0 + 1 < g.h, 0,
-                                             ColorFilter<LUT>::invert(filt), lut);
+  color_rows<1, true, StripPlanes, ONE, LUT, STD>(F, g, sp, eplanes, efr, y0, x0, !ONE && y0 + 1 < g.h, 0,
+                                                  ColorFilter<LUT>::invert(filt), lut);
 }
 
 
@@ -2428,9 +2526,6 @@
   for (int j = 0; j < 8; ++j) wsrow[j] = v[j];
 }
 
-#ifndef VF_ABL
-#define VF_ABL 0
-#endif
 template <bool FAST>
 __device__ __forceinline__ void fdct_pass1_planes(const uint8_t *plane, int pitch, int bx, int sy, bool real,
                                                   const uint4 &tw, const uint8_t *dummy, uint4 *s_tab,
@@ -2504,14 +2599,19 @@
 }
 
 constexpr uint32_t kFdctGroup = 8;
-template <int CH, int CV, bool FAST, bool PL>
+template <int CH, int CV, bool FAST, bool PL, bool STD = false>
 __global__ __launch_bounds__(256) __attribute__((amdgpu_waves_per_eu(8))) void k_fdct(const EncFrame *__restrict__ fr, const EncTables *tab, const uint8_t *pix,
                                               int16_t *dcq, uint32_t *acbits, uint32_t *acscr, int bgr) {
-  const EncFrame &F = fr[blockIdx.y];
+  static_assert(PL || !STD, "the fixed-geometry form reads the sample planes");
+  const EncFrame &F = fr[STD ? blockIdx.z : blockIdx.y];
   const Geom &g = F.g;
-  const uint32_t bpm = (uint32_t)g.bpm, nmcu = (uint32_t)g.nmcu;
+  const uint32_t bpm = STD ? 4u : (uint32_t)g.bpm, nmcu = (uint32_t)g.nmcu;
   const uint32_t ngroups = (nmcu + kFdctGroup - 1) / kFdctGroup;
-  if (blockIdx.x * 4 >= ngroups * bpm) return;
+  if constexpr (STD) {
+    if (blockIdx.x * kFdctGroup >= (uint32_t)g.mcux || blockIdx.y >= (uint32_t)g.mcuy) return;
+  } else {
+    if (blockIdx.x * 4 >= ngroups * bpm) return;
+  }
   __shared__ int32_t ws[32][8][9];
   __shared__ __attribute__((aligned(16))) uint32_t acw[32][kAcWords];
   __shared__ uint4 s_tab[192];
@@ -2524,13 +2624,20 @@
   const uint32_t (*const s_ac)[256] = reinterpret_cast<const uint32_t (*)[256]>(reinterpret_cast<const uint32_t *>(s_tab) + 256);
   const uint32_t slot = threadIdx.x >> 3, r = threadIdx.x & 7, lm = slot & (kFdctGroup - 1);
   int16_t *const qo = reinterpret_cast<int16_t *>(&ws[slot][0][0]);
-  const uint32_t unit = blockIdx.x * 4 + __builtin_amdgcn_readfirstlane(threadIdx.x >> 6);
-  const uint32_t grp = unit / bpm, c = unit - grp * bpm;
-  const uint32_t mcu = grp * kFdctGroup + lm;
-  const uint32_t b = mcu * bpm + c;
+  const uint32_t wave = __builtin_amdgcn_readfirstlane(threadIdx.x >> 6);
+  const uint32_t unit = blockIdx.x * 4 + wave;
+  const uint32_t grp = STD ? 0u : unit / bpm, c = STD ? wave : unit - grp * bpm;
+  uint32_t mcu = grp * kFdctGroup + lm;
   uint32_t k = 0, bx = 0, by = 0;
   bool real = false;
-  if (grp < ngroups) {
+  if constexpr (STD) {
+    const uint32_t mcux = (uint32_t)g.mcux, mx = blockIdx.x * kFdctGroup + lm;
+    k = c < 2 ? 0u : c - 1;
+    mcu = blockIdx.y * mcux + mx;
+    bx = c < 2 ? mx * 2 + c : mx;
+    by = blockIdx.y;
+    real = mx < mcux && bx < (uint32_t)g.wb[k];
+  } else if (grp < ngroups) {
     k = (uint32_t)g.bcomp[c];
     const uint32_t mcux = (uint32_t)g.mcux;
     uint32_t mx = (grp * kFdctGroup) % mcux + lm, my = (grp * kFdctGroup) / mcux;
@@ -2539,6 +2646,7 @@
     by = my * (uint32_t)g.mv[k] + (uint32_t)g.byo[c];
     real = mcu < nmcu && bx < (uint32_t)g.wb[k] && by < (uint32_t)g.hb[k];
   }
+  const uint32_t b = mcu * bpm + c;
   const uint8_t *img = pix + F.img_off;
   const uint8_t *dummy = reinterpret_cast<const uint8_t *>(tab->fdct_lds);
   {
@@ -3081,11 +3189,16 @@
 
 hipError_t dec_idct_color422(const DecFrame *__restrict__ fr, int n, int max_w, int max_h, const int16_t *coef,
                              const int32_t *dcseq, const uint8_t *nmask, uint8_t *eplanes, const EncFrame *efr,
-                             int invert, int one_row, hipStream_t s, const LutTable *lut) {
+                             int invert, int one_row, hipStream_t s, const LutTable *lut, int std422) {
   if (n <= 0 || max_w <= 0 || max_h <= 0) return hipSuccess;
   const unsigned mcux = (unsigned)((max_w + 15) / 16), mcuy = (unsigned)((max_h + 7) / 8);
   const dim3 grid((mcux + kStripMcus - 1) / kStripMcus, mcuy, (unsigned)n);
-  if (lut && one_row)
+  if (std422 && !one_row) return hipErrorInvalidValue;
+  if (std422 && lut)
+    hipLaunchKernelGGL((k_idct_color422<true, true, true>), grid, dim3(256), 0, s, fr, coef, dcseq, nmask, eplanes, efr, *lut);
+  else if (std422)
+    hipLaunchKernelGGL((k_idct_color422<true, false, true>), grid, dim3(256), 0, s, fr, coef, dcseq, nmask, eplanes, efr, invert);
+  else if (lut && one_row)
     hipLaunchKernelGGL((k_idct_color422<true, true>), grid, dim3(256), 0, s, fr, coef, dcseq, nmask, eplanes, efr, *lut);
   else if (lut)
     hipLaunchKernelGGL((k_idct_color422<false, true>), grid, dim3(256), 0, s, fr, coef, dcseq, nmask, eplanes, efr, *lut);
@@ -3098,8 +3211,14 @@
 
 hipError_t enc_fdct(const EncFrame *__restrict__ fr, int n, uint32_t max_blocks, const EncTables *tab, const uint8_t *pix,
                     int16_t *dcq, uint32_t *acbits, uint32_t *acscr, int bgr, int fastdct, int ch, int cv, int planes,
-                    hipStream_t s) {
+                    hipStream_t s, int std_w, int std_h) {
   if (n <= 0 || !max_blocks) return hipSuccess;
+  if (planes && std_w > 0 && std_h > 0) {
+    const dim3 grid(((unsigned)(std_w + 15) / 16 + kFdctGroup - 1) / kFdctGroup, (unsigned)(std_h + 7) / 8, (unsigned)n);
+    if (fastdct) hipLaunchKernelGGL((k_fdct<1, 1, true, true, true>), grid, dim3(256), 0, s, fr, tab, pix, dcq, acbits, acscr, bgr);
+    else hipLaunchKernelGGL((k_fdct<1, 1, false, true, true>), grid, dim3(256), 0, s, fr, tab, pix, dcq, acbits, acscr, bgr);
+    return hipGetLastError();
+  }
   const dim3 grid((max_blocks + 70 + 31) / 32, (unsigned)n);
   if (planes) {
     if (fastdct) hipLaunchKernelGGL((k_fdct<1, 1, true, true>), grid, dim3(256), 0, s, fr, tab, pix, dcq, acbits, acscr, bgr);
diff --git a/distributed-video-filter_amd/csrc/vf_jpeg_plan.h b/distributed-video-filter_amd/csrc/vf_jpeg_plan.h
--- a/distributed-video-filter_amd/csrc/vf_jpeg_plan.h
+++ b/distributed-video-filter_amd/csrc/vf_jpeg_plan.h
@@ -22,6 +22,7 @@
   const char *write4 = nullptr;
   const char *fuse = nullptr;
   const char *fuse_idct = nullptr;
+  const char *std422 = nullptr;
   const char *idct24 = nullptr;
   const char *fetch_learn = nullptr;
   const char *trace = nullptr;
@@ -39,6 +40,7 @@
     s.write4 = env_str("VF_JPEG_WRITE4");
     s.fuse = env_str("VF_JPEG_FUSE");
     s.fuse_idct = env_str("VF_JPEG_FUSE_IDCT");
+    s.std422 = env_str("VF_JPEG_STD422");
     s.idct24 = env_str("VF_JPEG_IDCT24");
     s.fetch_learn = env_str("VF_JPEG_FETCH_LEARN");
     s.trace = env_str("VF_JPEG_TRACE");
@@ -51,6 +53,7 @@
   bool tabs4 = true;
   bool pow2bpm = true;
   bool d422 = true;
+  bool e422 = false;
   uint32_t max_sub = 0;
   uint64_t bits_per_block = 0;
 };
@@ -66,6 +69,7 @@
   bool write4 = true;
   bool fuse = false;
   bool fuse_idct = false;
+  bool std422 = false;
   bool enc_fast = false;
   bool stats = false;
   bool trace = false;
@@ -93,6 +97,7 @@
   p.write4 = flag_on(sw.write4);
   p.fuse = fuse_requested && flag_on(sw.fuse);
   p.fuse_idct = p.fuse && t.d422 && flag_on(sw.fuse_idct);
+  p.std422 = p.fuse_idct && t.e422 && flag_on(sw.std422);
   p.stats = sw.sync_stats != nullptr;
   p.trace = sw.trace != nullptr;
   return p;
```
